# Gorilla-Lab-SCUT/frustum-convnet

Measured on AMD Instinct MI355X. Metric: frustums/sec (train fwd+bwd) KITTI-car B=32 N=1024, higher is better.
Workload: dtype f32 (fp32 operands split into two 16-bit parts, 3 MFMAs per product, fp32 accumulate); 1 GPU; cfgs/det_sample.yaml KITTI-car, batch=32/GPU, Npoint=1024, L=(280,140,70,35), train fwd+bwd+Adam; global_batch=32, parallelism=dp1

## Files before the change

frustum_convnet_amd/_native.py:

```python
import ctypes
import os

_HERE = os.path.dirname(os.path.abspath(__file__))
LIB_PATH = os.path.join(_HERE, os.environ.get("FCN_LIB_NAME", "libfcn_hip.so"))

c_fp = ctypes.c_void_p

BN_RUNNING = 0
BN_TRAIN = 1
BN_FROZEN = 2


class PnDesc(ctypes.Structure):
    _fields_ = [("B", ctypes.c_int32), ("N", ctypes.c_int32), ("L", ctypes.c_int32), ("K", ctypes.c_int32),
                ("C1", ctypes.c_int32), ("C2", ctypes.c_int32), ("C3", ctypes.c_int32),
                ("nvec", ctypes.c_int32), ("training", ctypes.c_int32),
                ("eps", ctypes.c_float), ("momentum", ctypes.c_float), ("nlc", ctypes.c_int32),
                ("precision", ctypes.c_int32), ("grouped", ctypes.c_int32)]


CN_MAXLEV = 5
CN_MAXLAYER = 18


class CnDesc(ctypes.Structure):
    _fields_ = [("B", ctypes.c_int32), ("L", ctypes.c_int32 * CN_MAXLEV), ("nvec", ctypes.c_int32),
                ("reg_out", ctypes.c_int32), ("training", ctypes.c_int32),
                ("eps", ctypes.c_float), ("momentum", ctypes.c_float), ("prepacked", ctypes.c_int32),
                ("precision", ctypes.c_int32), ("nlev", ctypes.c_int32), ("c1", ctypes.c_int32)]


class CnParams(ctypes.Structure):
    _fields_ = [("W", c_fp * CN_MAXLAYER), ("gamma", c_fp * CN_MAXLAYER), ("beta", c_fp * CN_MAXLAYER),
                ("running_mean", c_fp * CN_MAXLAYER), ("running_var", c_fp * CN_MAXLAYER),
                ("num_batches_tracked", c_fp * CN_MAXLAYER), ("bias", c_fp)]


class CnWs(ctypes.Structure):
    _fields_ = [("y", c_fp), ("dz", c_fp), ("wp", c_fp), ("bn", c_fp), ("stat", c_fp), ("bstat", c_fp),
                ("coef", c_fp), ("partial", c_fp), ("oh64", c_fp), ("flags", c_fp)]


class PnParams(ctypes.Structure):
    _fields_ = [("W", c_fp * 3), ("gamma", c_fp * 3), ("beta", c_fp * 3),
                ("running_mean", c_fp * 3), ("running_var", c_fp * 3), ("num_batches_tracked", c_fp * 3)]


class PnWs(ctypes.Structure):
    _fields_ = [("woff", c_fp), ("ent", c_fp), ("ewin", c_fp), ("tiles", c_fp), ("y2", c_fp), ("y3", c_fp), ("amax", c_fp),
                ("stat", c_fp), ("bn", c_fp), ("gmax", c_fp), ("dy3", c_fp), ("dz2", c_fp), ("bstat", c_fp),
                ("coef", c_fp), ("partial", c_fp), ("nsplit", ctypes.c_int32), ("gmom", c_fp), ("wenc", c_fp), ("flags", c_fp), ("pkey", c_fp),
                ("partial_both", ctypes.c_int32)]


class PnInferWs(ctypes.Structure):
    _fields_ = [("w1f", c_fp), ("wenc", c_fp), ("shift", c_fp)]


class InpDesc(ctypes.Structure):
    _fields_ = [("B", ctypes.c_int32), ("N", ctypes.c_int32), ("pt_stride", ctypes.c_int32), ("L", ctypes.c_int32 * 4),
                ("stride", ctypes.c_double * 4), ("max_depth", ctypes.c_double),
                ("random_flip", ctypes.c_int32), ("random_shift", ctypes.c_int32)]


class Inp5Desc(ctypes.Structure):
    _fields_ = [("B", ctypes.c_int32), ("N", ctypes.c_int32), ("pt_stride", ctypes.c_int32), ("L", ctypes.c_int32 * 5),
                ("stride", ctypes.c_double * 5), ("max_depth", ctypes.c_double),
                ("random_flip", ctypes.c_int32), ("random_shift", ctypes.c_int32)]


class InpRefineDesc(ctypes.Structure):
    _fields_ = [("B", ctypes.c_int32), ("N", ctypes.c_int32), ("pt_stride", ctypes.c_int32), ("Lpad", ctypes.c_int32 * 4),
                ("stride", ctypes.c_double * 4), ("random_flip", ctypes.c_int32), ("random_shift", ctypes.c_int32)]


EXPORTS = ("fcn_arch", "fcn_build_hash", "fcn_stat_replicas", "fcn_query_depth_point_f32", "fcn_query_depth_point_multi_f32", "fcn_pn_wgrad_rows", "fcn_pn_compact", "fcn_pn_group_compact", "fcn_pn_group_compact2",
           "fcn_pn_pack_weights", "fcn_pn_pack_weights_all", "fcn_pn_infer_fold", "fcn_pn_infer", "fcn_pn_forward", "fcn_pn_backward", "fcn_pn_backward2", "fcn_pn_backward3", "fcn_pn_backward_dense", "fcn_pn_conv_fwd", "fcn_det_loss_tail", "fcn_det_loss_tail_rows", "fcn_det_loss_tail_rows2", "fcn_det_iou_metrics",
           "fcn_det_loss_tail_scratch_floats", "fcn_adam_step_f32", "fcn_sgd_step_f32", "fcn_adam_step_slots", "fcn_prepare_inputs", "fcn_prepare_inputs_refine", "fcn_prepare_inputs_sunrgbd", "fcn_stamp", "fcn_stream_capture_id",
           "fcn_convnet_sizes", "fcn_convnet_logits_ld", "fcn_convnet_pack", "fcn_convnet_forward", "fcn_convnet_forward2",
           "fcn_convnet_backward", "fcn_box3d_iou_pair_f32", "fcn_decode_detections", "fcn_rotate_nms_3d")

_lib = None


FLAG_NONFINITE = 1


class NativeError(RuntimeError):
    pass


def lib():
    global _lib
    if _lib is not None:
        return _lib
    if not os.path.exists(LIB_PATH):
        raise ImportError(
            "frustum_convnet_amd: %s not found -- build it with `python -m frustum_convnet_amd.build` "
            "(hipcc --offload-arch=gfx950). There is no CPU/PyTorch fallback for the hot path." % LIB_PATH)
    import torch
    L = ctypes.CDLL(LIB_PATH)
    L.fcn_arch.restype = ctypes.c_int
    if hasattr(L, "fcn_build_hash"):
        L.fcn_build_hash.restype = ctypes.c_char_p
        L.fcn_build_hash.argtypes = []
    L.fcn_arch.argtypes = []
    L.fcn_pn_wgrad_rows.restype = ctypes.c_int
    L.fcn_pn_wgrad_rows.argtypes = []
    if hasattr(L, "fcn_stat_replicas"):
        L.fcn_stat_replicas.restype = ctypes.c_int
        L.fcn_stat_replicas.argtypes = []
    L.fcn_query_depth_point_f32.restype = ctypes.c_int
    L.fcn_query_depth_point_f32.argtypes = [
        c_fp, ctypes.c_int64, ctypes.c_int64, c_fp, ctypes.c_int64, ctypes.c_int64,
        ctypes.c_int, ctypes.c_int, ctypes.c_int, ctypes.c_float, ctypes.c_int, c_fp, c_fp, c_fp]
    if hasattr(L, "fcn_query_depth_point_multi_f32"):
        L.fcn_query_depth_point_multi_f32.restype = ctypes.c_int
        L.fcn_query_depth_point_multi_f32.argtypes = [ctypes.c_int, c_fp, ctypes.c_int64, ctypes.c_int64, c_fp, c_fp, c_fp,
                                                      ctypes.c_int, ctypes.c_int, c_fp, c_fp, c_fp, c_fp, c_fp, c_fp]
    L.fcn_pn_compact.restype = ctypes.c_int
    L.fcn_pn_compact.argtypes = [ctypes.POINTER(PnDesc), c_fp, c_fp, c_fp, c_fp, ctypes.POINTER(PnWs), c_fp]
    L.fcn_pn_group_compact.restype = ctypes.c_int
    L.fcn_pn_group_compact.argtypes = [ctypes.c_int, c_fp, c_fp, c_fp, c_fp, c_fp, c_fp, c_fp, c_fp]
    L.fcn_pn_group_compact2.restype = ctypes.c_int
    L.fcn_pn_group_compact2.argtypes = [ctypes.c_int, c_fp, c_fp, c_fp, c_fp, c_fp, c_fp, c_fp, ctypes.c_int, c_fp]
    if hasattr(L, "fcn_pn_pack_weights") or "FCN_LIB_NAME" not in os.environ:
        L.fcn_pn_pack_weights.restype = ctypes.c_int
        L.fcn_pn_pack_weights.argtypes = [ctypes.POINTER(PnDesc), ctypes.POINTER(PnParams), ctypes.POINTER(PnWs), c_fp]
        L.fcn_pn_pack_weights_all.restype = ctypes.c_int
        L.fcn_pn_pack_weights_all.argtypes = [ctypes.c_int, c_fp, c_fp, c_fp, c_fp]
    L.fcn_pn_forward.restype = ctypes.c_int
    L.fcn_pn_forward.argtypes = [ctypes.POINTER(PnDesc), ctypes.POINTER(PnParams), c_fp, c_fp,
                                 ctypes.POINTER(PnWs), c_fp, c_fp]
    if hasattr(L, "fcn_pn_infer") or "FCN_LIB_NAME" not in os.environ:
        L.fcn_pn_infer_fold.restype = ctypes.c_int
        L.fcn_pn_infer_fold.argtypes = [ctypes.c_int, c_fp, c_fp, c_fp, c_fp, c_fp]
        L.fcn_pn_infer.restype = ctypes.c_int
        L.fcn_pn_infer.argtypes = [ctypes.POINTER(PnDesc), c_fp, c_fp, ctypes.POINTER(PnWs), ctypes.POINTER(PnInferWs), c_fp, c_fp]
    L.fcn_pn_backward.restype = ctypes.c_int
    L.fcn_pn_backward.argtypes = [ctypes.POINTER(PnDesc), ctypes.POINTER(PnParams), c_fp,
                                  ctypes.POINTER(PnWs), c_fp * 3, c_fp * 3, c_fp * 3, c_fp]
    L.fcn_pn_backward2.restype = ctypes.c_int
    L.fcn_pn_backward2.argtypes = [ctypes.POINTER(PnDesc), ctypes.POINTER(PnParams), c_fp,
                                   ctypes.POINTER(PnWs), c_fp * 3, c_fp * 3, c_fp * 3, c_fp, c_fp, ctypes.POINTER(c_fp)]
    if hasattr(L, "fcn_pn_backward3"):
        L.fcn_pn_backward3.restype = ctypes.c_int
        L.fcn_pn_backward3.argtypes = [ctypes.POINTER(PnDesc), ctypes.POINTER(PnParams), c_fp,
                                       ctypes.POINTER(PnWs), c_fp * 3, c_fp * 3, c_fp * 3, c_fp, c_fp, c_fp, ctypes.POINTER(c_fp)]
    if hasattr(L, "fcn_pn_backward_dense"):
        L.fcn_pn_backward_dense.restype = ctypes.c_int
        L.fcn_pn_backward_dense.argtypes = [ctypes.POINTER(PnDesc), ctypes.POINTER(PnParams), c_fp,
                                            ctypes.POINTER(PnWs), c_fp * 3, c_fp * 3, c_fp * 3, c_fp]
    L.fcn_pn_conv_fwd.restype = ctypes.c_int
    L.fcn_pn_conv_fwd.argtypes = [ctypes.POINTER(PnDesc), ctypes.POINTER(PnParams), ctypes.POINTER(PnWs),
                                  ctypes.c_int, ctypes.c_int, c_fp]
    L.fcn_det_loss_tail.restype = ctypes.c_int
    L.fcn_det_loss_tail.argtypes = [c_fp] * 9 + [ctypes.c_int] * 4 + [ctypes.c_float] * 4 + [c_fp] * 4
    L.fcn_adam_step_f32.restype = ctypes.c_int
    L.fcn_adam_step_f32.argtypes = [c_fp] * 4 + [ctypes.c_int64] + [c_fp] * 3
    L.fcn_sgd_step_f32.restype = ctypes.c_int
    L.fcn_sgd_step_f32.argtypes = [c_fp] * 3 + [ctypes.c_int64] + [c_fp] * 2
    L.fcn_prepare_inputs.restype = ctypes.c_int
    L.fcn_prepare_inputs.argtypes = [ctypes.POINTER(InpDesc)] + [c_fp] * 13 + [c_fp * 4] + [c_fp] * 7
    L.fcn_prepare_inputs_sunrgbd.restype = ctypes.c_int
    L.fcn_prepare_inputs_sunrgbd.argtypes = [ctypes.POINTER(Inp5Desc)] + [c_fp] * 15 + [c_fp * 5] + [c_fp] * 7
    L.fcn_prepare_inputs_refine.restype = ctypes.c_int
    L.fcn_prepare_inputs_refine.argtypes = [ctypes.POINTER(InpRefineDesc)] + [c_fp] * 12 + [c_fp * 4] + [c_fp] * 8
    L.fcn_stamp.restype = ctypes.c_int
    L.fcn_stamp.argtypes = [c_fp, c_fp]
    L.fcn_stream_capture_id.restype = ctypes.c_int
    L.fcn_stream_capture_id.argtypes = [c_fp, ctypes.POINTER(ctypes.c_uint64)]
    L.fcn_adam_step_slots.restype = ctypes.c_int64
    L.fcn_adam_step_slots.argtypes = [ctypes.c_int64]
    L.fcn_det_loss_tail_rows.restype = ctypes.c_int
    L.fcn_det_loss_tail_rows.argtypes = [c_fp] * 8 + [ctypes.c_int] * 4 + [ctypes.c_float] * 4 + [c_fp] * 3
    L.fcn_det_loss_tail_rows2.restype = ctypes.c_int
    L.fcn_det_loss_tail_rows2.argtypes = [c_fp] * 8 + [ctypes.c_int] * 4 + [ctypes.c_float] * 4 + [c_fp] * 5
    L.fcn_det_iou_metrics.restype = ctypes.c_int
    L.fcn_det_iou_metrics.argtypes = [c_fp, ctypes.c_int] + [c_fp] * 6 + [ctypes.c_int] * 4 + [ctypes.c_float] + [c_fp] * 3
    L.fcn_det_loss_tail_scratch_floats.restype = ctypes.c_int
    L.fcn_det_loss_tail_scratch_floats.argtypes = [ctypes.c_int, ctypes.c_int]
    L.fcn_convnet_sizes.restype = ctypes.c_int
    L.fcn_convnet_sizes.argtypes = [ctypes.POINTER(CnDesc), ctypes.POINTER(ctypes.c_int64 * 6)]
    L.fcn_convnet_logits_ld.restype = ctypes.c_int
    L.fcn_convnet_logits_ld.argtypes = [ctypes.POINTER(CnDesc)]
    L.fcn_convnet_pack.restype = ctypes.c_int
    L.fcn_convnet_pack.argtypes = [ctypes.POINTER(CnDesc), ctypes.POINTER(CnParams), ctypes.POINTER(CnWs), c_fp, c_fp]
    L.fcn_convnet_forward.restype = ctypes.c_int
    L.fcn_convnet_forward.argtypes = [ctypes.POINTER(CnDesc), ctypes.POINTER(CnParams), ctypes.POINTER(CnWs),
                                      c_fp * CN_MAXLEV, c_fp, c_fp, c_fp]
    L.fcn_convnet_forward2.restype = ctypes.c_int
    L.fcn_convnet_forward2.argtypes = [ctypes.POINTER(CnDesc), ctypes.POINTER(CnParams), ctypes.POINTER(CnWs),
                                       c_fp * CN_MAXLEV, c_fp, c_fp, c_fp, ctypes.POINTER(c_fp)]
    L.fcn_convnet_backward.restype = ctypes.c_int
    L.fcn_convnet_backward.argtypes = [ctypes.POINTER(CnDesc), ctypes.POINTER(CnParams), ctypes.POINTER(CnWs),
                                       c_fp * CN_MAXLEV, c_fp, c_fp, c_fp * CN_MAXLEV, c_fp * CN_MAXLAYER, c_fp * CN_MAXLAYER,
                                       c_fp * CN_MAXLAYER, c_fp, c_fp, c_fp, ctypes.POINTER(c_fp)]
    L.fcn_box3d_iou_pair_f32.restype = ctypes.c_int
    L.fcn_box3d_iou_pair_f32.argtypes = [c_fp, c_fp, ctypes.c_int, c_fp, c_fp]
    L.fcn_decode_detections.restype = ctypes.c_int
    L.fcn_decode_detections.argtypes = [c_fp, ctypes.c_int] + [c_fp] * 5 + [ctypes.c_int] * 5 + [c_fp] * 3
    L.fcn_rotate_nms_3d.restype = ctypes.c_int
    L.fcn_rotate_nms_3d.argtypes = [c_fp] * 3 + [ctypes.c_int] * 3 + [ctypes.c_float, ctypes.c_int] + [c_fp] * 3
    _lib = L
    return L


def check(rc, what):
    if rc != 0:
        raise NativeError("%s failed with code %d (hipError_t or FCN_E_*; see include/fcn_hip.h)" % (what, rc))


def ptr(t):
    return None if t is None else ctypes.c_void_p(t.data_ptr())


def current_stream(device=None):
    import torch
    return ctypes.c_void_p(torch.cuda.current_stream(device).cuda_stream)


_unknown_capture = [0]


def capture_id(device=None):
    import torch
    if not torch.cuda.is_available() or not torch.cuda.is_current_stream_capturing():
        return 0
    cid = ctypes.c_uint64(0)
    rc = lib().fcn_stream_capture_id(current_stream(device), ctypes.byref(cid))
    if rc != 0 or cid.value == 0:
        _unknown_capture[0] -= 1
        return _unknown_capture[0]
    return int(cid.value)
```

frustum_convnet_amd/build.py:

```python
import os
import subprocess
import sys

HERE = os.path.dirname(os.path.abspath(__file__))
CSRC = os.path.join(HERE, "csrc")
SOURCES = ["grouping.hip", "group_compact.hip", "pointnet_fwd.hip", "pointnet_bwd.hip", "loss_tail.hip", "fcn_net.hip", "optim.hip", "inputs.hip", "box_iou.hip"]
HEADERS = ["fcn_common.h", "fcn_tuning.h", "gemm_tile.h", "pn_pack.h", "pn_infer.h", "box_iou.h", os.path.join("..", "..", "include", "fcn_hip.h")]
LIB = os.path.join(HERE, "libfcn_hip.so")
FLAGS = ["--offload-arch=gfx950", "-O3", "-std=c++17", "-fPIC", "-shared", "-fno-fast-math",
         "-ffp-contract=off"]


OBJ = os.path.join(CSRC, "_obj")


def source_hash(extra_flags=()):
    import hashlib
    h = hashlib.sha256()
    for name in SOURCES + HEADERS:
        with open(os.path.join(CSRC, name), "rb") as f:
            h.update(name.encode() + b"\0" + f.read() + b"\0")
    h.update(" ".join(FLAGS + list(extra_flags)).encode())
    return h.hexdigest()[:16]


def _deps_mtime():
    return max(os.path.getmtime(os.path.join(CSRC, h)) for h in HEADERS + [os.path.abspath(__file__)])


def _stale():
    if not os.path.exists(LIB):
        return True
    t = os.path.getmtime(LIB)
    deps = [os.path.join(CSRC, s) for s in SOURCES + HEADERS] + [os.path.abspath(__file__)]
    return any(os.path.getmtime(d) > t for d in deps)


def build(force=False, verbose=True, lib=None, extra_flags=()):
    variant = lib is not None or bool(extra_flags)
    lib = lib or LIB
    if not force and not variant and not _stale():
        return lib
    from concurrent.futures import ThreadPoolExecutor
    hipcc = os.environ.get("HIPCC", "/opt/rocm/bin/hipcc")
    cflags = [f for f in FLAGS if f != "-shared"] + list(extra_flags)
    objdir = OBJ + ("_variant_%d" % os.getpid() if variant else "")
    os.makedirs(objdir, exist_ok=True)
    hdr_t = _deps_mtime()

    def compile_one(src):
        path, obj = os.path.join(CSRC, src), os.path.join(objdir, src.replace(".hip", ".o"))
        if not force and not variant and os.path.exists(obj) and os.path.getmtime(obj) > max(os.path.getmtime(path), hdr_t):
            return obj
        cmd = [hipcc] + cflags + ["-c", path, "-o", obj]
        if verbose:
            print("[fcn build]", " ".join(cmd), flush=True)
        subprocess.check_call(cmd)
        return obj

    with ThreadPoolExecutor(max_workers=min(len(SOURCES), os.cpu_count() or 4)) as ex:
        objs = list(ex.map(compile_one, SOURCES))
    hsrc, hobj = os.path.join(objdir, "build_hash.cpp"), os.path.join(objdir, "build_hash.o")
    with open(hsrc, "w") as f:
        f.write('extern "C" const char *fcn_build_hash(void) { return "%s"; }\n' % source_hash(extra_flags))
    import shutil
    cxx = os.environ.get("CXX") or shutil.which("g++") or shutil.which("c++")
    if cxx:
        subprocess.check_call([cxx, "-O1", "-fPIC", "-c", hsrc, "-o", hobj])
    else:
        subprocess.check_call([hipcc, "-x", "c++", "-O1", "-fPIC", "-c", hsrc, "-o", hobj])
    objs.append(hobj)
    cmd = [hipcc, "--offload-arch=gfx950", "-shared", "-fPIC"] + objs + ["-o", lib]
    if verbose:
        print("[fcn build]", " ".join(cmd), flush=True)
    subprocess.check_call(cmd)
    if variant:
        shutil.rmtree(objdir, ignore_errors=True)
    return lib


if __name__ == "__main__":
    build(force="--force" in sys.argv)
```

frustum_convnet_amd/csrc/box_iou.hip:

```cpp
#include "fcn_common.h"
#define FCN_HD __device__ __forceinline__
#include "box_iou.h"

__global__ void iou_pair_kernel(const float *__restrict__ c1, const float *__restrict__ c2, int n, float *__restrict__ out)
{
    const int i = blockIdx.x * blockDim.x + threadIdx.x;
    if (i >= n) return;
    const float *a = c1 + (int64_t)i * 24, *b = c2 + (int64_t)i * 24;
    const int ord[4] = {6, 7, 4, 5};
    float ax[4], az[4], bx[4], bz[4];
#pragma unroll
    for (int k = 0; k < 4; ++k) {
        ax[k] = a[ord[k] * 3]; az[k] = a[ord[k] * 3 + 2];
        bx[k] = b[ord[k] * 3]; bz[k] = b[ord[k] * 3 + 2];
    }
    float i2, i3;
    fcn_iou_from_polys(ax, az, a[1], a[13], bx, bz, b[1], b[13], &i2, &i3);
    out[2 * i] = i2;
    out[2 * i + 1] = i3;
}

extern "C" int fcn_box3d_iou_pair_f32(const float *corners1, const float *corners2, int n, float *out2, void *stream)
{
    if (n < 0 || (n > 0 && (!corners1 || !corners2 || !out2))) return FCN_E_BADARG;
    if (n == 0) return 0;
    hipLaunchKernelGGL(iou_pair_kernel, dim3((n + 127) / 128), dim3(128), 0, (hipStream_t)stream, corners1, corners2, n, out2);
    FCN_CHECK_LAUNCH();
    return 0;
}

#define IOM_T 128

struct IouMetricArgs {
    const float *logits;
    const int64_t *cls_label;
    const float *ref2;
    const float *box_center, *box_heading, *box_size;
    const float *mean_size;
    float *scratch;
    float *out4;
    int B, L2, ld, nb, ns;
    float thresh;
};

__global__ __launch_bounds__(IOM_T) void iou_metric_kernel(IouMetricArgs a)
{
    __shared__ float sh[4][IOM_T / 64];
    const int tid = threadIdx.x, lane = tid & 63, wave = tid >> 6;
    const int R = a.B * a.L2, nb = a.nb, ns = a.ns;
    const int r = blockIdx.x * IOM_T + tid;
    float s2 = 0.f, s3 = 0.f, st = 0.f, sn = 0.f;
    if (r < R && a.cls_label[r] == 1) {
        const int b = r / a.L2, l = r % a.L2;
        const float *o = a.logits + (int64_t)r * a.ld + 2;
        const float per = 6.283185307179586f / (float)nb, half = per * 0.5f;
        int ah = 0, as = 0;
        float mx = o[3];
        for (int j = 1; j < nb; ++j)
            if (o[3 + j] > mx) { mx = o[3 + j]; ah = j; }
        const float *ss = o + 3 + 2 * nb;
        mx = ss[0];
        for (int j = 1; j < ns; ++j)
            if (ss[j] > mx) { mx = ss[j]; as = j; }
        float pa = (float)ah * per + o[3 + nb + ah] * half;
        if (pa > 3.141592653589793f) pa -= 6.283185307179586f;
        const float *sr3 = o + 3 + 2 * nb + ns + 3 * as;
        const float m0 = a.mean_size[as * 3], m1 = a.mean_size[as * 3 + 1], m2 = a.mean_size[as * 3 + 2];
        const float pcx = o[0] + a.ref2[((int64_t)b * 3 + 0) * a.L2 + l], pcy = o[1] + a.ref2[((int64_t)b * 3 + 1) * a.L2 + l],
                    pcz = o[2] + a.ref2[((int64_t)b * 3 + 2) * a.L2 + l];
        const float hl = a.box_heading[b];
        float i2, i3;
        fcn_iou_from_params(pcx, pcy, pcz, sr3[0] * m0 + m0, sr3[1] * m1 + m1, sr3[2] * m2 + m2, cosf(pa), sinf(pa),
                            a.box_center[b * 3], a.box_center[b * 3 + 1], a.box_center[b * 3 + 2], a.box_size[b * 3],
                            a.box_size[b * 3 + 1], a.box_size[b * 3 + 2], cosf(hl), sinf(hl), &i2, &i3);
        s2 = i2; s3 = i3; st = (i3 >= a.thresh) ? 1.f : 0.f; sn = 1.f;
    }
    s2 = wave_sum_f32(s2); s3 = wave_sum_f32(s3); st = wave_sum_f32(st); sn = wave_sum_f32(sn);
    if (lane == 0) { sh[0][wave] = s2; sh[1][wave] = s3; sh[2][wave] = st; sh[3][wave] = sn; }
    __syncthreads();
    if (tid == 0) {
        float t[4];
        for (int q = 0; q < 4; ++q) {
            t[q] = 0.f;
            for (int w = 0; w < IOM_T / 64; ++w) t[q] += sh[q][w];
            if (t[q] != 0.f) atomicAdd(&a.scratch[q], t[q]);
        }
        __threadfence();
        const int ticket = atomicAdd((int *)&a.scratch[4], 1);
        if (ticket == (int)gridDim.x - 1) {
            __threadfence();
            float v[4];
            for (int q = 0; q < 4; ++q) v[q] = __hip_atomic_load(&a.scratch[q], __ATOMIC_RELAXED, __HIP_MEMORY_SCOPE_AGENT);
            const float inv = v[3] > 0.f ? 1.f / v[3] : 0.f;
            a.out4[0] = v[0] * inv; a.out4[1] = v[1] * inv; a.out4[2] = v[2] * inv; a.out4[3] = v[3];
            for (int q = 0; q < 4; ++q) a.scratch[q] = 0.f;
            ((int *)a.scratch)[4] = 0;
        }
    }
}

extern "C" int fcn_det_iou_metrics(const float *logits, int ld, const int64_t *cls_label, const float *center_ref2,
                                   const float *box3d_center, const float *box3d_heading, const float *box3d_size,
                                   const float *mean_size, int B, int L2, int num_heading_bin, int num_size_cluster,
                                   float iou_thresh, float *scratch8, float *out4, void *stream)
{
    if (!logits || !cls_label || !center_ref2 || !box3d_center || !box3d_heading || !box3d_size || !mean_size || !scratch8 ||
        !out4)
        return FCN_E_BADARG;
    if (B <= 0 || L2 <= 0 || num_heading_bin < 1 || num_size_cluster < 1) return FCN_E_BADARG;
    if (ld < 2 + 3 + 2 * num_heading_bin + 4 * num_size_cluster) return FCN_E_BADARG;
    IouMetricArgs a;
    a.logits = logits; a.cls_label = cls_label; a.ref2 = center_ref2; a.box_center = box3d_center;
    a.box_heading = box3d_heading; a.box_size = box3d_size; a.mean_size = mean_size; a.scratch = scratch8; a.out4 = out4;
    a.B = B; a.L2 = L2; a.ld = ld; a.nb = num_heading_bin; a.ns = num_size_cluster; a.thresh = iou_thresh;
    hipLaunchKernelGGL(iou_metric_kernel, dim3((B * L2 + IOM_T - 1) / IOM_T), dim3(IOM_T), 0, (hipStream_t)stream, a);
    FCN_CHECK_LAUNCH();
    return 0;
}

#define DEC_T 256
#define DEC_NB_MAX 16
#define DEC_NS_MAX 8

struct DecodeArgs {
    const float *logits;
    const float *ref2;
    const float *mean_size;
    const float *rot_angle;
    const float *ref_center;
    const float *rgb_prob;
    float *dets;
    int32_t *valid;
    int B, L2, ld, nb, ns, method;
};

__global__ __launch_bounds__(DEC_T) void decode_kernel(DecodeArgs a)
{
    __shared__ float best_s[DEC_T];
    __shared__ int best_i[DEC_T];
    __shared__ int nfg_s;
    const int b = blockIdx.x, tid = threadIdx.x;
    const int L2 = a.L2, nb = a.nb, ns = a.ns;
    if (tid == 0) nfg_s = 0;
    __syncthreads();
    float bs = -1.f;
    int bi = 0x7fffffff, cnt = 0;
    for (int l = tid; l < L2; l += DEC_T) {
        const float *row = a.logits + ((int64_t)b * L2 + l) * a.ld;
        const float c0 = row[0], c1 = row[1];
        const float m = fmaxf(c0, c1), e0 = expf(c0 - m), e1 = expf(c1 - m);
        const float p0 = e0 / (e0 + e1), p1 = e1 / (e0 + e1);
        cnt += (p0 < p1) ? 1 : 0;
        if (p1 > bs) { bs = p1; bi = l; }
    }
    best_s[tid] = bs;
    best_i[tid] = bi;
    if (cnt) atomicAdd(&nfg_s, cnt);
    __syncthreads();
    for (int o = DEC_T / 2; o > 0; o >>= 1) {
        if (tid < o) {
            const float s2 = best_s[tid + o];
            const int i2 = best_i[tid + o];
            if (s2 > best_s[tid] || (s2 == best_s[tid] && i2 < best_i[tid])) { best_s[tid] = s2; best_i[tid] = i2; }
        }
        __syncthreads();
    }
    const bool use_top = (a.method == 0) || (nfg_s == 0);
    const int top = best_i[0];
    const float rot = a.rot_angle[b];
    const float cr = cosf(-rot), sr = sinf(-rot);
    const float rcx = a.ref_center ? a.ref_center[b * 3] : 0.f, rcy = a.ref_center ? a.ref_center[b * 3 + 1] : 0.f,
                rcz = a.ref_center ? a.ref_center[b * 3 + 2] : 0.f;
    const float rgb = a.rgb_prob ? a.rgb_prob[b] : 1.f;
    const float per = 6.283185307179586f / (float)nb, half = per * 0.5f;
    for (int l = tid; l < L2; l += DEC_T) {
        const int64_t r = (int64_t)b * L2 + l;
        const float *row = a.logits + r * a.ld;
        const float c0 = row[0], c1 = row[1];
        const float m = fmaxf(c0, c1), e0 = expf(c0 - m), e1 = expf(c1 - m);
        const float p0 = e0 / (e0 + e1), p1 = e1 / (e0 + e1);
        const bool sel = use_top ? (l == top) : (p0 < p1);
        const float *o = row + 2;
        int ah = 0, as = 0;
        float mx = o[3];
        for (int j = 1; j < nb; ++j)
            if (o[3 + j] > mx) { mx = o[3 + j]; ah = j; }
        const float *ss = o + 3 + 2 * nb;
        mx = ss[0];
        for (int j = 1; j < ns; ++j)
            if (ss[j] > mx) { mx = ss[j]; as = j; }
        float ang = (float)ah * per + o[3 + nb + ah] * half;
        if (ang > 3.141592653589793f) ang -= 6.283185307179586f;
        const float *sr3 = o + 3 + 2 * nb + ns + 3 * as;
        const float sl = sr3[0] * a.mean_size[as * 3] + a.mean_size[as * 3];
        const float sw = sr3[1] * a.mean_size[as * 3 + 1] + a.mean_size[as * 3 + 1];
        const float sh = sr3[2] * a.mean_size[as * 3 + 2] + a.mean_size[as * 3 + 2];
        const float cx = o[0] + a.ref2[((int64_t)b * 3 + 0) * L2 + l], cy = o[1] + a.ref2[((int64_t)b * 3 + 1) * L2 + l],
                    cz = o[2] + a.ref2[((int64_t)b * 3 + 2) * L2 + l];
        const float tx = cr * cx - sr * cz + rcx;
        const float tz = sr * cx + cr * cz + rcz;
        const float ty = cy + rcy + 0.5f * sh;
        float *d = a.dets + r * 8;
        d[0] = tx; d[1] = ty; d[2] = tz; d[3] = sl; d[4] = sw; d[5] = sh; d[6] = ang + rot; d[7] = p1 + rgb;
        a.valid[r] = (sel && !(sh < 0.01f || sw < 0.01f || sl < 0.01f)) ? 1 : 0;
    }
}

extern "C" int fcn_decode_detections(const float *logits, int ld, const float *center_ref2, const float *mean_size,
                                     const float *rot_angle, const float *ref_center, const float *rgb_prob, int B, int L2,
                                     int num_heading_bin, int num_size_cluster, int method, float *dets, int32_t *valid,
                                     void *stream)
{
    if (!logits || !center_ref2 || !mean_size || !rot_angle || !dets || !valid) return FCN_E_BADARG;
    if (B <= 0 || L2 <= 0 || num_heading_bin < 1 || num_size_cluster < 1) return FCN_E_BADARG;
    if (ld < 2 + 3 + 2 * num_heading_bin + 4 * num_size_cluster) return FCN_E_BADARG;
    if (method != 0 && method != 1) return FCN_E_BADARG;
    DecodeArgs a;
    a.logits = logits; a.ref2 = center_ref2; a.mean_size = mean_size; a.rot_angle = rot_angle; a.ref_center = ref_center;
    a.rgb_prob = rgb_prob; a.dets = dets; a.valid = valid; a.B = B; a.L2 = L2; a.ld = ld; a.nb = num_heading_bin;
    a.ns = num_size_cluster; a.method = method;
    hipLaunchKernelGGL(decode_kernel, dim3(B), dim3(DEC_T), 0, (hipStream_t)stream, a);
    FCN_CHECK_LAUNCH();
    return 0;
}

#define NMS_T 256
#define NMS_MAXC 4096

struct NmsArgs {
    const float *dets;
    const int32_t *valid;
    const int32_t *unit_group;
    int U, rows_per_unit, G, top_k;
    float thresh;
    int32_t *keep;
    int32_t *keep_cnt;
};

struct NmsBox {
    float x[4], z[4], ytop, ybot, lo[3], hi[3];
};

__device__ __forceinline__ void nms_load(const float *d, NmsBox &b)
{
    const float co = cosf(d[6]), si = sinf(d[6]);
    fcn_bev_rect(d[0], d[2], d[3], d[4], co, si, b.x, b.z);
    b.ytop = d[1] + 0.5f * d[5];
    b.ybot = d[1] - 0.5f * d[5];
    b.lo[0] = fminf(fminf(b.x[0], b.x[1]), fminf(b.x[2], b.x[3]));
    b.hi[0] = fmaxf(fmaxf(b.x[0], b.x[1]), fmaxf(b.x[2], b.x[3]));
    b.lo[2] = fminf(fminf(b.z[0], b.z[1]), fminf(b.z[2], b.z[3]));
    b.hi[2] = fmaxf(fmaxf(b.z[0], b.z[1]), fmaxf(b.z[2], b.z[3]));
    b.lo[1] = b.ybot;
    b.hi[1] = b.ytop;
}

__global__ __launch_bounds__(NMS_T) void nms_kernel(NmsArgs a)
{
    __shared__ float key[NMS_MAXC];
    __shared__ int32_t row[NMS_MAXC];
    __shared__ unsigned char dead[NMS_MAXC];
    __shared__ int n_s, cur_s, kept_s;
    const int g = blockIdx.x, tid = threadIdx.x;
    if (tid == 0) { n_s = 0; kept_s = 0; }
    __syncthreads();
    for (int u = 0; u < a.U; ++u) {
        if (a.unit_group[u] != g) continue;
        for (int base = 0; base < a.rows_per_unit; base += NMS_T) {
            const int l = base + tid;
            const int r = u * a.rows_per_unit + l;
            const bool ok = l < a.rows_per_unit && (!a.valid || a.valid[r] != 0);
            const unsigned long long mask = __ballot(ok);
            const int lane = tid & 63, wave = tid >> 6;
            __shared__ int wcnt[NMS_T / 64];
            if (lane == 0) wcnt[wave] = __popcll(mask);
            __syncthreads();
            int off = n_s;
            for (int w = 0; w < wave; ++w) off += wcnt[w];
            const int pos = off + __popcll(mask & ((1ull << lane) - 1ull));
            if (ok && pos < NMS_MAXC) { key[pos] = a.dets[(int64_t)r * 8 + 7]; row[pos] = r; }
            __syncthreads();
            if (tid == 0) {
                int t = 0;
                for (int w = 0; w < NMS_T / 64; ++w) t += wcnt[w];
                n_s += t;
            }
            __syncthreads();
        }
    }
    const int n = n_s;
    if (n > NMS_MAXC) {
        if (tid == 0) a.keep_cnt[g] = -1;
        return;
    }
    int np2 = 1;
    while (np2 < n) np2 <<= 1;
    for (int i = n + tid; i < np2; i += NMS_T) { key[i] = -INFINITY; row[i] = -1; }
    for (int i = tid; i < np2; i += NMS_T) dead[i] = 0;
    __syncthreads();
    for (int k = 2; k <= np2; k <<= 1) {
        for (int j = k >> 1; j > 0; j >>= 1) {
            for (int i = tid; i < np2; i += NMS_T) {
                const int p = i ^ j;
                if (p > i) {
                    const bool desc = (i & k) == 0;
                    const float ki = key[i], kp = key[p];
                    const int ri = row[i], rp = row[p];
                    const bool i_first = (ki > kp) || (ki == kp && ri > rp);
                    if (desc ? !i_first : i_first) { key[i] = kp; key[p] = ki; row[i] = rp; row[p] = ri; }
                }
            }
            __syncthreads();
        }
    }
    int i = 0;
    while (true) {
        if (tid == 0) {
            int c = i;
            while (c < n && dead[c]) ++c;
            cur_s = c;
            if (c < n) {
                if (kept_s < a.top_k) a.keep[(int64_t)g * a.top_k + kept_s] = row[c];
                kept_s += 1;
            }
        }
        __syncthreads();
        const int c = cur_s;
        if (c >= n) break;
        NmsBox bi;
        nms_load(a.dets + (int64_t)row[c] * 8, bi);
        for (int j = c + 1 + tid; j < n; j += NMS_T) {
            if (dead[j]) continue;
            NmsBox bj;
            nms_load(a.dets + (int64_t)row[j] * 8, bj);
            bool apart = false;
#pragma unroll
            for (int q = 0; q < 3; ++q) apart = apart || (fminf(bi.hi[q], bj.hi[q]) - fmaxf(bi.lo[q], bj.lo[q]) <= 0.f);
            if (apart) continue;
            float i2, i3;
            fcn_iou_from_polys(bi.x, bi.z, bi.ytop, bi.ybot, bj.x, bj.z, bj.ytop, bj.ybot, &i2, &i3);
            if (i3 >= a.thresh) dead[j] = 1;
        }
        i = c + 1;
        __syncthreads();
    }
    if (tid == 0) a.keep_cnt[g] = kept_s < a.top_k ? kept_s : a.top_k;
}

extern "C" int fcn_rotate_nms_3d(const float *dets, const int32_t *valid, const int32_t *unit_group, int num_units,
                                 int rows_per_unit, int num_groups, float thresh, int top_k, int32_t *keep,
                                 int32_t *keep_cnt, void *stream)
{
    if (!dets || !unit_group || !keep || !keep_cnt) return FCN_E_BADARG;
    if (num_units <= 0 || rows_per_unit <= 0 || num_groups <= 0 || top_k <= 0) return FCN_E_BADARG;
    NmsArgs a;
    a.dets = dets; a.valid = valid; a.unit_group = unit_group; a.U = num_units; a.rows_per_unit = rows_per_unit;
    a.G = num_groups; a.top_k = top_k; a.thresh = thresh; a.keep = keep; a.keep_cnt = keep_cnt;
    hipLaunchKernelGGL(nms_kernel, dim3(num_groups), dim3(NMS_T), 0, (hipStream_t)stream, a);
    FCN_CHECK_LAUNCH();
    return 0;
}
```

frustum_convnet_amd/csrc/loss_tail.hip:

```cpp
#include "fcn_common.h"

#define LT_NB 12
#define LT_MIN_THREADS 64

struct LossArgs {
    const float *cls_raw;
    const float *reg_raw;
    const int64_t *cls_label;
    const float *ref2;
    const float *box_center;
    const float *box_heading;
    const float *box_size;
    const int64_t *size_class;
    const float *mean_size;
    float *out;
    float *dcls;
    float *dreg;
    int B, L2;
    float w_box, w_corner, w_headreg, w_sizereg;
    int ld;
    float *scratch;
    float *total;
};

template <int NT, int N>
__device__ __forceinline__ void block_sums(float (&v)[N], float *sh)
{
    const int lane = threadIdx.x & 63, wave = threadIdx.x >> 6;
#pragma unroll
    for (int i = 0; i < N; ++i) v[i] = wave_sum_f32(v[i]);
    __syncthreads();
    if (lane == 0) {
#pragma unroll
        for (int i = 0; i < N; ++i) sh[wave * N + i] = v[i];
    }
    __syncthreads();
#pragma unroll
    for (int i = 0; i < N; ++i) {
        float t = 0.f;
        for (int w = 0; w < NT / 64; ++w) t += sh[w * N + i];
        v[i] = t;
    }
}

__device__ __forceinline__ float pymod(float a, float b) { return a - b * floorf(a / b); }

__device__ __forceinline__ void corners8(float cx, float cy, float cz, float c, float s, float l, float w, float h,
                                         float (&px)[8], float (&py)[8], float (&pz)[8])
{
#pragma unroll
    for (int k = 0; k < 8; ++k) {
        const float sx = (k & 2) ? -0.5f : 0.5f;
        const float sy = (k & 4) ? -0.5f : 0.5f;
        const float sz = ((k & 3) == 1 || (k & 3) == 2) ? -0.5f : 0.5f;
        const float x = sx * l, y = sy * h, z = sz * w;
        px[k] = c * x + s * z + cx;
        py[k] = y + cy;
        pz[k] = -s * x + c * z + cz;
    }
}

template <int NS, int LT_THREADS>
__global__ __launch_bounds__(LT_THREADS) void loss_tail_kernel(LossArgs a)
{
    constexpr int NB = LT_NB, NC = 3 + 2 * NB + 4 * NS;
    constexpr int SW = (NC + 2) | 1;
    __shared__ float shN[LT_THREADS / 64 * 11];
    __shared__ int last_s;
    __shared__ float gS[LT_THREADS * SW];
    __shared__ float gG[LT_THREADS * SW];
    const int tid = threadIdx.x;
    const int B = a.B, L2 = a.L2, R = B * L2;
    const float TWO_PI = 6.283185307179586f, PI = 3.141592653589793f;
    const float per = (float)(6.283185307179586 / NB), half = (float)(6.283185307179586 / NB / 2.0);

    typedef float lt_v4f __attribute__((ext_vector_type(4)));
    typedef const lt_v4f __attribute__((address_space(1))) *lt_gv4fp;
    constexpr int LT_NV = 16;
    const int row0 = blockIdx.x * LT_THREADS;
    const int nrow = min(LT_THREADS, R - row0);
    const int q4 = a.ld >> 2;
    const int sh_q = a.ld == 128 ? 5 : 4;
    const int nbatch = a.ld ? (q4 + LT_NV - 1) / LT_NV : 0;
    lt_v4f lv[LT_NV];
#define LT_LOAD_BATCH(bt)                                                                                             \
    _Pragma("unroll") for (int k = 0; k < LT_NV; ++k) {                                                               \
        const int i = tid + LT_THREADS * (k + LT_NV * (bt));                                                          \
        const int rr = min(i >> sh_q, nrow - 1), c4 = i & (q4 - 1);              \
        lv[k] = *(lt_gv4fp)(a.cls_raw + (int64_t)(row0 + rr) * a.ld + 4 * c4);                                        \
    }
#define LT_STAGE_BATCH(bt)                                                                                            \
    _Pragma("unroll") for (int k = 0; k < LT_NV; ++k) {                                                               \
        const int i = tid + LT_THREADS * (k + LT_NV * (bt));                                                          \
        const int rr = i >> sh_q, c4 = i & (q4 - 1);                                                                  \
        if (rr < nrow) {                                                                                              \
            _Pragma("unroll") for (int j = 0; j < 4; ++j)                                                             \
                if (4 * c4 + j < NC + 2) gS[rr * SW + 4 * c4 + j] = lv[k][j];                                         \
        }                                                                                                             \
    }
    if (a.ld) LT_LOAD_BATCH(0);

    float cfg_ = 0.f, ckeep = 0.f;
    {
        typedef long long lt_v2l __attribute__((ext_vector_type(2)));
        typedef const lt_v2l __attribute__((address_space(1))) *lt_gv2lp;
        const int R2 = R >> 1;
        constexpr int LT_CNT = 18;
        for (int base = 0; base < R2; base += LT_CNT * LT_THREADS) {
            lt_v2l lab[LT_CNT];
#pragma unroll
            for (int k = 0; k < LT_CNT; ++k) lab[k] = *(lt_gv2lp)(a.cls_label + 2 * min(base + tid + k * LT_THREADS, R2 - 1));
#pragma unroll
            for (int k = 0; k < LT_CNT; ++k) {
                const bool in = base + tid + k * LT_THREADS < R2;
                cfg_ += in ? ((lab[k][0] == 1) ? 1.f : 0.f) + ((lab[k][1] == 1) ? 1.f : 0.f) : 0.f;
                ckeep += in ? ((lab[k][0] != -1) ? 1.f : 0.f) + ((lab[k][1] != -1) ? 1.f : 0.f) : 0.f;
            }
        }
        if ((R & 1) && tid == 0) {
            const int64_t lab = a.cls_label[R - 1];
            cfg_ += (lab == 1) ? 1.f : 0.f;
            ckeep += (lab != -1) ? 1.f : 0.f;
        }
    }
    float cnt2[2] = {cfg_, ckeep};
    block_sums<LT_THREADS, 2>(cnt2, shN);
    const float nfg = cnt2[0], nkeep = cnt2[1];
    const float inv_cls = 1.f / (nfg + 1e-14f);
    const float inv_fg = nfg > 0.f ? 1.f / nfg : 0.f;

    float acc[11];
#pragma unroll
    for (int i = 0; i < 11; ++i) acc[i] = 0.f;

    if (a.ld) {
        LT_STAGE_BATCH(0);
        if (nbatch > 1) {
            LT_LOAD_BATCH(1);
            LT_STAGE_BATCH(1);
        }
        __syncthreads();
    }

    for (int r = blockIdx.x * LT_THREADS + tid; r < R; r += gridDim.x * LT_THREADS) {
        const int b = r / L2, l = r % L2;
        const int64_t lab = a.cls_label[r];
        const float c0 = a.ld ? gS[tid * SW] : a.cls_raw[((int64_t)b * 2 + 0) * L2 + l];
        const float c1 = a.ld ? gS[tid * SW + 1] : a.cls_raw[((int64_t)b * 2 + 1) * L2 + l];
        const float m = fmaxf(c0, c1);
        const float e0 = expf(c0 - m), e1 = expf(c1 - m);
        const float p0 = e0 / (e0 + e1), p1 = e1 / (e0 + e1);
        float g0 = 0.f, g1 = 0.f;
        if (lab != -1) {
            const int t = lab >= 1 ? 1 : 0;
            const float pt = t ? p1 : p0;
            const float alpha = t ? 0.25f : 0.75f;
            const float om = 1.f - pt, lg = logf(pt + 1e-14f);
            acc[1] += -alpha * om * om * lg;
            const float dpt = -alpha * (-2.f * om * lg + om * om / (pt + 1e-14f));
            const float gt_ = dpt * pt * om * inv_cls;
            g0 = t ? -gt_ : gt_;
            g1 = t ? gt_ : -gt_;
            acc[8] += ((p1 > p0 ? 1 : 0) == t) ? 1.f : 0.f;
        }
        if (a.dcls) {
            if (a.ld) {
                gG[tid * SW] = g0;
                gG[tid * SW + 1] = g1;
            } else {
                a.dcls[((int64_t)b * 2 + 0) * L2 + l] = g0;
                a.dcls[((int64_t)b * 2 + 1) * L2 + l] = g1;
            }
        }
        float *go = gG + tid * SW + 2;
#pragma unroll
        for (int j = 0; j < NC; ++j) go[j] = 0.f;
        if (lab == 1) {
            if (!a.ld) {
#pragma unroll
                for (int j = 0; j < NC; ++j) gS[tid * SW + 2 + j] = a.reg_raw[((int64_t)b * NC + j) * L2 + l];
            }
            const float *o = gS + tid * SW + 2;
            const float rx = a.ref2[((int64_t)b * 3 + 0) * L2 + l], ry = a.ref2[((int64_t)b * 3 + 1) * L2 + l],
                        rz = a.ref2[((int64_t)b * 3 + 2) * L2 + l];
            const float clx = a.box_center[b * 3], cly = a.box_center[b * 3 + 1], clz = a.box_center[b * 3 + 2];
            const float hlab = a.box_heading[b];
            const float sl0 = a.box_size[b * 3], sl1 = a.box_size[b * 3 + 1], sl2 = a.box_size[b * 3 + 2];
            const int sc = min(max((int)a.size_class[b], 0), NS - 1);
            const float ex0 = a.mean_size[sc * 3], ex1 = a.mean_size[sc * 3 + 1], ex2 = a.mean_size[sc * 3 + 2];
            const float wB = a.w_box * inv_fg;

            {
                const float dx = clx - rx - o[0], dy = cly - ry - o[1], dz = clz - rz - o[2];
                const float dist = sqrtf(dx * dx + dy * dy + dz * dz);
                const float q = fminf(dist, 3.f);
                acc[2] += 0.5f * q * q + 3.f * (dist - q);
                if (dist > 0.f) {
                    const float k = -wB * q / dist;
                    go[0] += k * dx; go[1] += k * dy; go[2] += k * dz;
                }
            }
            const float ga = pymod(hlab, TWO_PI);
            const float shifted = pymod(ga + half, TWO_PI);
            int hc = (int)floorf(shifted / per);
            hc = hc < 0 ? 0 : (hc > NB - 1 ? NB - 1 : hc);
            const float hres = (shifted - ((float)hc * per + half)) / half;
            {
                float mx = o[3];
                int am = 0;
#pragma unroll
                for (int j = 1; j < NB; ++j)
                    if (o[3 + j] > mx) { mx = o[3 + j]; am = j; }
                float se = 0.f, ej[NB];
#pragma unroll
                for (int j = 0; j < NB; ++j) { ej[j] = expf(o[3 + j] - mx); se += ej[j]; }
                acc[3] += logf(se) + mx - o[3 + hc];
#pragma unroll
                for (int j = 0; j < NB; ++j) go[3 + j] += wB * (ej[j] / se - (j == hc ? 1.f : 0.f));
                acc[9] += (am == hc) ? 1.f : 0.f;
                const float e = o[3 + NB + hc] - hres;
                const float ab = fabsf(e), q = fminf(ab, 1.f);
                acc[4] += 0.5f * q * q + (ab - q);
                go[3 + NB + hc] += wB * a.w_headreg * (e > 0.f ? q : (e < 0.f ? -q : 0.f));
            }
            {
                const float *ss = &o[3 + 2 * NB];
                float mx = ss[0];
                int am = 0;
#pragma unroll
                for (int j = 1; j < NS; ++j)
                    if (ss[j] > mx) { mx = ss[j]; am = j; }
                float se = 0.f;
#pragma unroll
                for (int j = 0; j < NS; ++j) {
                    const float ej = expf(ss[j] - mx);
                    go[3 + 2 * NB + j] = ej;
                    se += ej;
                }
                acc[5] += logf(se) + mx - ss[sc];
#pragma unroll
                for (int j = 0; j < NS; ++j) go[3 + 2 * NB + j] = wB * (go[3 + 2 * NB + j] / se - (j == sc ? 1.f : 0.f));
                acc[10] += (am == sc) ? 1.f : 0.f;
            }
            const int so = 3 + 2 * NB + NS + sc * 3;
            {
                const float v0 = (sl0 - ex0) / ex0 - o[so], v1 = (sl1 - ex1) / ex1 - o[so + 1],
                            v2 = (sl2 - ex2) / ex2 - o[so + 2];
                const float n = sqrtf(v0 * v0 + v1 * v1 + v2 * v2);
                const float q = fminf(n, 1.f);
                acc[6] += 0.5f * q * q + (n - q);
                if (n > 0.f) {
                    const float k = -wB * a.w_sizereg * q / n;
                    go[so] += k * v0; go[so + 1] += k * v1; go[so + 2] += k * v2;
                }
            }
            {
                float ang = (float)hc * per + o[3 + NB + hc] * half;
                if (ang > PI) ang -= TWO_PI;
                const float pl = o[so] * ex0 + ex0, pw = o[so + 1] * ex1 + ex1, ph = o[so + 2] * ex2 + ex2;
                const float pcx = rx + o[0], pcy = ry + o[1], pcz = rz + o[2];
                float px[8], py[8], pz[8], gx[8], gy[8], gz[8], fx[8], fy[8], fz[8];
                const float c = cosf(ang), s = sinf(ang);
                const float hf = hlab + PI;
                corners8(pcx, pcy, pcz, c, s, pl, pw, ph, px, py, pz);
                corners8(clx, cly, clz, cosf(hlab), sinf(hlab), sl0, sl1, sl2, gx, gy, gz);
                corners8(clx, cly, clz, cosf(hf), sinf(hf), sl0, sl1, sl2, fx, fy, fz);
                float d1 = 0.f, d2 = 0.f;
#pragma unroll
                for (int k = 0; k < 8; ++k) {
                    d1 += sqrtf((px[k] - gx[k]) * (px[k] - gx[k]) + (py[k] - gy[k]) * (py[k] - gy[k]) +
                                (pz[k] - gz[k]) * (pz[k] - gz[k]));
                    d2 += sqrtf((px[k] - fx[k]) * (px[k] - fx[k]) + (py[k] - fy[k]) * (py[k] - fy[k]) +
                                (pz[k] - fz[k]) * (pz[k] - fz[k]));
                }
                d1 *= 0.125f; d2 *= 0.125f;
                const bool first = d1 <= d2;
                const float cd = first ? d1 : d2;
                const float q = fminf(cd, 1.f);
                acc[7] += 0.5f * q * q + (cd - q);
                const float wk = wB * a.w_corner * q * 0.125f;
                float dcx = 0.f, dcy = 0.f, dcz = 0.f, dl = 0.f, dw = 0.f, dh = 0.f, dang = 0.f;
#pragma unroll
                for (int k = 0; k < 8; ++k) {
                    const float tx = first ? gx[k] : fx[k], ty = first ? gy[k] : fy[k], tz = first ? gz[k] : fz[k];
                    const float ex_ = px[k] - tx, ey_ = py[k] - ty, ez_ = pz[k] - tz;
                    const float nn = sqrtf(ex_ * ex_ + ey_ * ey_ + ez_ * ez_);
                    if (nn > 0.f) {
                        const float kx = wk * ex_ / nn, ky = wk * ey_ / nn, kz = wk * ez_ / nn;
                        const float sx = (k & 2) ? -0.5f : 0.5f, sy = (k & 4) ? -0.5f : 0.5f;
                        const float sz = ((k & 3) == 1 || (k & 3) == 2) ? -0.5f : 0.5f;
                        const float x = sx * pl, z = sz * pw;
                        dcx += kx; dcy += ky; dcz += kz;
                        dl += kx * c * sx - kz * s * sx;
                        dw += kx * s * sz + kz * c * sz;
                        dh += ky * sy;
                        dang += kx * (-s * x + c * z) + kz * (-c * x - s * z);
                    }
                }
                go[0] += dcx; go[1] += dcy; go[2] += dcz;
                go[so] += dl * ex0; go[so + 1] += dw * ex1; go[so + 2] += dh * ex2;
                go[3 + NB + hc] += dang * half;
            }
        }
        if (a.ld) {
        } else if (a.dreg) {
#pragma unroll
            for (int j = 0; j < NC; ++j) a.dreg[((int64_t)b * NC + j) * L2 + l] = go[j];
        }
    }
    if (a.ld && a.dcls) {
        __syncthreads();
        for (int i = tid; i < nrow * q4; i += LT_THREADS) {
            const int rr = i >> sh_q, c4 = i & (q4 - 1);
            lt_v4f v;
#pragma unroll
            for (int j = 0; j < 4; ++j) v[j] = 4 * c4 + j < NC + 2 ? gG[rr * SW + 4 * c4 + j] : 0.f;
            *(lt_v4f *)(a.dcls + (int64_t)(row0 + rr) * a.ld + 4 * c4) = v;
        }
    }
    float tot[11];
#pragma unroll
    for (int i = 0; i < 11; ++i) tot[i] = acc[i];
    block_sums<LT_THREADS, 11>(tot, shN);
    if (tid == 0) {
        int ticket;
        if (a.scratch) {
#pragma unroll
            for (int i = 1; i < 11; ++i) a.scratch[32 + 16 * blockIdx.x + i] = tot[i];
            __threadfence();
            ticket = atomicAdd((int *)a.scratch, 1);
        } else {
#pragma unroll
            for (int i = 1; i < 11; ++i) atomicAdd(&a.out[i], tot[i]);
            __threadfence();
            ticket = atomicAdd((int *)&a.out[15], 1);
        }
        last_s = (ticket == (int)gridDim.x - 1) ? 1 : 0;
    }
    __syncthreads();
    if (last_s && a.scratch) {
        __threadfence();
        float pt_[11];
#pragma unroll
        for (int i = 1; i < 11; ++i) pt_[i] = 0.f;
        for (int g = tid; g < (int)gridDim.x; g += LT_THREADS)
#pragma unroll
            for (int i = 1; i < 11; ++i)
                pt_[i] += __hip_atomic_load(&a.scratch[32 + 16 * g + i], __ATOMIC_RELAXED, __HIP_MEMORY_SCOPE_AGENT);
#pragma unroll
        for (int i = 1; i < 11; ++i) gG[tid * 11 + i] = pt_[i];
    }
    __syncthreads();
    if (last_s && tid == 0) {
        float t[11];
        if (a.scratch) {
#pragma unroll
            for (int i = 1; i < 11; ++i) t[i] = 0.f;
            const int nth = min((int)gridDim.x, LT_THREADS);
            for (int g = 0; g < nth; ++g)
#pragma unroll
                for (int i = 1; i < 11; ++i) t[i] += gG[g * 11 + i];
            ((int *)a.scratch)[0] = 0;
        } else {
            __threadfence();
#pragma unroll
            for (int i = 1; i < 11; ++i) t[i] = __hip_atomic_load(&a.out[i], __ATOMIC_RELAXED, __HIP_MEMORY_SCOPE_AGENT);
        }
        const float cls = t[1] * inv_cls;
        const float center = t[2] * inv_fg, hcls = t[3] * inv_fg, hres = t[4] * inv_fg;
        const float scls = t[5] * inv_fg, sres = t[6] * inv_fg, corner = t[7] * inv_fg;
        const float total = cls + a.w_box * (center + hcls + scls + a.w_headreg * hres + a.w_sizereg * sres + a.w_corner * corner);
        a.out[0] = total;
        a.out[1] = cls; a.out[2] = center; a.out[3] = hcls; a.out[4] = hres;
        a.out[5] = scls; a.out[6] = sres; a.out[7] = corner;
        a.out[8] = nkeep > 0.f ? t[8] / nkeep : 0.f; a.out[9] = t[9] * inv_fg; a.out[10] = t[10] * inv_fg;
        a.out[11] = nfg;
        a.out[12] = a.out[13] = a.out[14] = a.out[15] = 0.f;
        if (a.total) a.total[0] = total;
    }
}

static int launch_loss(const LossArgs &a, int ns, hipStream_t st)
{
    if (!a.scratch) {
        hipError_t e = hipMemsetAsync(a.out, 0, 16 * sizeof(float), st);
        if (e != hipSuccess) return (int)e;
    }
    const int R = a.B * a.L2;
    if (ns == 3) hipLaunchKernelGGL((loss_tail_kernel<3, 128>), dim3((R + 127) / 128), dim3(128), 0, st, a);
    else hipLaunchKernelGGL((loss_tail_kernel<10, 64>), dim3((R + 63) / 64), dim3(64), 0, st, a);
    FCN_CHECK_LAUNCH();
    return 0;
}

extern "C" int fcn_det_loss_tail(const float *cls_raw, const float *reg_raw, const int64_t *cls_label,
                                 const float *center_ref2, const float *box3d_center, const float *box3d_heading,
                                 const float *box3d_size, const int64_t *size_class, const float *mean_size,
                                 int B, int L2, int num_heading_bin, int num_size_cluster,
                                 float w_box, float w_corner, float w_headreg, float w_sizereg,
                                 float *out16, float *dcls, float *dreg, void *stream)
{
    if (!cls_raw || !reg_raw || !cls_label || !center_ref2 || !box3d_center || !box3d_heading || !box3d_size ||
        !size_class || !mean_size || !out16)
        return FCN_E_BADARG;
    if (num_heading_bin != LT_NB || (num_size_cluster != 3 && num_size_cluster != 10)) return FCN_E_LIMIT;
    if (B <= 0 || L2 <= 0) return FCN_E_BADARG;
    if ((uintptr_t)cls_label & 15) return FCN_E_BADARG;
    LossArgs a;
    a.cls_raw = cls_raw; a.reg_raw = reg_raw; a.cls_label = cls_label; a.ref2 = center_ref2;
    a.box_center = box3d_center; a.box_heading = box3d_heading; a.box_size = box3d_size; a.size_class = size_class;
    a.mean_size = mean_size; a.out = out16; a.dcls = dcls; a.dreg = dreg; a.B = B; a.L2 = L2;
    a.w_box = w_box; a.w_corner = w_corner; a.w_headreg = w_headreg; a.w_sizereg = w_sizereg; a.ld = 0;
    a.scratch = nullptr; a.total = nullptr;
    return launch_loss(a, num_size_cluster, (hipStream_t)stream);
}

extern "C" int fcn_det_loss_tail_rows2(const float *logits, const int64_t *cls_label, const float *center_ref2,
                                       const float *box3d_center, const float *box3d_heading, const float *box3d_size,
                                       const int64_t *size_class, const float *mean_size, int B, int L2,
                                       int num_heading_bin, int num_size_cluster,
                                       float w_box, float w_corner, float w_headreg, float w_sizereg,
                                       float *out16, float *dlogits, float *scratch, float *total, void *stream);

extern "C" int fcn_det_loss_tail_rows(const float *logits, const int64_t *cls_label, const float *center_ref2,
                                      const float *box3d_center, const float *box3d_heading, const float *box3d_size,
                                      const int64_t *size_class, const float *mean_size, int B, int L2,
                                      int num_heading_bin, int num_size_cluster,
                                      float w_box, float w_corner, float w_headreg, float w_sizereg,
                                      float *out16, float *dlogits, void *stream)
{
    return fcn_det_loss_tail_rows2(logits, cls_label, center_ref2, box3d_center, box3d_heading, box3d_size, size_class,
                                   mean_size, B, L2, num_heading_bin, num_size_cluster, w_box, w_corner, w_headreg,
                                   w_sizereg, out16, dlogits, nullptr, nullptr, stream);
}

extern "C" int fcn_det_loss_tail_scratch_floats(int B, int L2)
{
    return (B <= 0 || L2 <= 0) ? 0 : 32 + 16 * ((B * L2 + LT_MIN_THREADS - 1) / LT_MIN_THREADS);
}

extern "C" int fcn_det_loss_tail_rows2(const float *logits, const int64_t *cls_label, const float *center_ref2,
                                       const float *box3d_center, const float *box3d_heading, const float *box3d_size,
                                       const int64_t *size_class, const float *mean_size, int B, int L2,
                                       int num_heading_bin, int num_size_cluster,
                                       float w_box, float w_corner, float w_headreg, float w_sizereg,
                                       float *out16, float *dlogits, float *scratch, float *total, void *stream)
{
    if (!logits || !cls_label || !center_ref2 || !box3d_center || !box3d_heading || !box3d_size || !size_class ||
        !mean_size || !out16)
        return FCN_E_BADARG;
    if (num_heading_bin != LT_NB || (num_size_cluster != 3 && num_size_cluster != 10)) return FCN_E_LIMIT;
    if (B <= 0 || L2 <= 0) return FCN_E_BADARG;
    if (((uintptr_t)cls_label & 15) || ((uintptr_t)logits & 15) || ((uintptr_t)dlogits & 15)) return FCN_E_BADARG;
    LossArgs a;
    a.cls_raw = logits; a.reg_raw = nullptr; a.cls_label = cls_label; a.ref2 = center_ref2;
    a.box_center = box3d_center; a.box_heading = box3d_heading; a.box_size = box3d_size; a.size_class = size_class;
    a.mean_size = mean_size; a.out = out16; a.dcls = dlogits; a.dreg = nullptr; a.B = B; a.L2 = L2;
    a.w_box = w_box; a.w_corner = w_corner; a.w_headreg = w_headreg; a.w_sizereg = w_sizereg;
    a.ld = (2 + 3 + 2 * num_heading_bin + 4 * num_size_cluster <= 64) ? 64 : 128;
    a.scratch = scratch; a.total = total;
    return launch_loss(a, num_size_cluster, (hipStream_t)stream);
}
```

frustum_convnet_amd/det_base.py:

```python
import math

import numpy as np
import os

import torch
import torch.nn as nn
import torch.nn.functional as F

from .config import cfg
from .dataset_info import DATASET_INFO
from .common import Conv1d, Conv2d, DeConv1d, init_params, softmax_focal_loss_ignore, get_accuracy, masked_mean, bn_momentum
from .query_depth_point import QueryDepthPoint
from .pointnet_fused import WorkspacePool, pointnet_pooled, launch_pooled, attach_pooled
from . import box_ops
from . import _native


def _bn_mode(module):
    if getattr(module, "bn_frozen", False):
        return _native.BN_FROZEN
    return _native.BN_TRAIN if module.training else _native.BN_RUNNING


class PointNetModule(nn.Module):

    def __init__(self, Infea, mlp, dist, nsample, use_xyz=True, use_feature=True):
        super(PointNetModule, self).__init__()
        self.dist = dist
        self.nsample = nsample
        self.use_xyz = use_xyz
        self.use_feature = Infea > 0
        if self.use_feature or not use_xyz:
            raise NotImplementedError(
                "only the xyz-only path (Infea == 0) is implemented: every shipped cfg has "
                "WITH_EXTRA_FEAT False and train_net_det.py:296 makes Infea <= 0 otherwise")
        self.query_depth_point = QueryDepthPoint(dist, nsample)
        self.conv1 = Conv2d(Infea + 3, mlp[0], 1)
        self.conv2 = Conv2d(mlp[0], mlp[1], 1)
        self.conv3 = Conv2d(mlp[1], mlp[2], 1)
        init_params([self.conv1[0], self.conv2[0], self.conv3[0]], 'kaiming_normal')
        init_params([self.conv1[1], self.conv2[1], self.conv3[1]], 1)
        self._pool = WorkspacePool()
        self.bn_frozen = False
        self.fused_eval = os.environ.get("FCN_FUSED_EVAL", "0") != "0"

    def fuse_eval(self, flag=True):
        self.fused_eval = bool(flag)
        return self

    def freeze_bn(self, flag=True):
        self.bn_frozen = bool(flag)
        return self

    def _param_pack(self):
        convs = (self.conv1, self.conv2, self.conv3)
        params = []
        for c in convs:
            params += [c[0].weight, c[1].weight, c[1].bias]
        bufs = ([c[1].running_mean for c in convs], [c[1].running_var for c in convs],
                [c[1].num_batches_tracked for c in convs])
        return params, bufs

    def forward_pooled(self, pc, new_pc, one_hot_vec=None, nlc=False):
        params, bufs = self._param_pack()
        bn = self.conv1[1]
        feat, _, _ = pointnet_pooled(self._pool, self.dist, self.nsample, _bn_mode(self), bn.eps,
                                     bn_momentum(bn),
                                     pc.contiguous(), new_pc.contiguous(), one_hot_vec, bufs, params, nlc=nlc,
                                     fuse_eval=self.fused_eval)
        return feat

    def launch_pooled(self, pc, new_pc, one_hot_vec=None, nlc=False):
        params, bufs = self._param_pack()
        bn = self.conv1[1]
        return launch_pooled(self._pool, self.dist, self.nsample, _bn_mode(self), bn.eps,
                             bn_momentum(bn),
                             pc.contiguous(), new_pc.contiguous(), one_hot_vec, bufs, params, nlc=nlc,
                             fuse_eval=self.fused_eval)

    def prepare_pooled(self, pc, new_pc, one_hot_vec=None, nlc=False):
        from .pointnet_fused import prepare_pooled
        params, bufs = self._param_pack()
        bn = self.conv1[1]
        return prepare_pooled(self._pool, self.dist, self.nsample, _bn_mode(self), bn.eps, bn_momentum(bn),
                              pc.contiguous(), new_pc.contiguous(), one_hot_vec, bufs, params, nlc=nlc,
                              fuse_eval=self.fused_eval)

    def attach_pooled(self, handle):
        feat, _, _ = attach_pooled(self._pool, handle)
        return feat

    def front_signature(self, nlc=False):
        from .pointnet_fused import _cfg_tuple
        from . import precision as _precision
        params, bufs = self._param_pack()
        bn = self.conv1[1]
        cfgt = _cfg_tuple(self.dist, self.nsample, _bn_mode(self), bn.eps, bn_momentum(bn), params, nlc, self.fused_eval)
        return (cfgt, _precision.code(), tuple(t.data_ptr() for t in params), tuple(t.data_ptr() for b in bufs for t in b))

    def forward(self, pc, feat, new_pc=None):
        from .pointnet_fused import dense_from_entries, dense_pointnet
        params, bufs = self._param_pack()
        bn = self.conv1[1]
        if pc.requires_grad and torch.is_grad_enabled():
            raise RuntimeError("PointNetModule.forward: no gradient w.r.t. the point cloud (the reference never asks for one either: "
                               "its inputs do not require grad)")
        mode = _bn_mode(self)
        if torch.is_grad_enabled() and any(p.requires_grad for p in params):
            if mode == _native.BN_RUNNING:
                raise NotImplementedError(
                    "PointNetModule.forward in eval mode with gradients enabled and trainable parameters: the backward of "
                    "running-statistics BatchNorm is not implemented; wrap the call in torch.no_grad() (inference), call "
                    ".train() (training) or .freeze_bn() (fine-tuning through the running statistics)")
            return dense_pointnet(self._pool, self.dist, self.nsample, mode, bn.eps, bn_momentum(bn),
                                  pc.contiguous(), new_pc.contiguous(), bufs, params)
        with torch.no_grad():
            return dense_from_entries(self._pool, self.dist, self.nsample, mode, bn.eps,
                                      bn_momentum(bn),
                                      pc.contiguous(), new_pc.contiguous(), bufs, params)


class PointNetFeat(nn.Module):

    SCALES = (([64, 64, 128], 32), ([64, 64, 128], 64), ([128, 128, 256], 64), ([256, 256, 512], 128))

    def __init__(self, input_channel=3, num_vec=0):
        super(PointNetFeat, self).__init__()
        self.num_vec = num_vec
        u = cfg.DATA.HEIGHT_HALF
        assert len(u) == len(self.SCALES)
        self.num_scales = len(self.SCALES)
        for i, (mlp, nsample) in enumerate(self.SCALES):
            setattr(self, "pointnet%d" % (i + 1),
                    PointNetModule(input_channel - 3, list(mlp), u[i], nsample, use_xyz=True, use_feature=True))
        self.concurrent_scales = True
        self.fused_front = os.environ.get("FCN_FUSED_FRONT", "1") != "0"
        self._stream_cache = {}
        self._prefetched = None
        self.set_wgrad_streams((self.num_scales - 1,))
        self.bwd_share = dict(self.BWD_SHARE.get(self.num_scales, ()))
        self.share_active = False
        self._step_id = 0

    def set_wgrad_streams(self, scales, three=False):
        for k, net in enumerate(self.nets):
            net._pool.side_wgrad = k in tuple(scales)
            net._pool.side_three = bool(three) and k in tuple(scales)

    BWD_SHARE = {4: ((1, 2),), 5: ((0, 2), (1, 3))}

    def share_backward_stream(self, scale, host):
        ns = self.num_scales
        if host is None:
            self.bwd_share.pop(scale, None)
            return
        if not (0 <= scale < host < ns - 1):
            raise ValueError("share_backward_stream: need 0 <= scale < host < %d (got scale %d, host %d)" % (ns - 1, scale, host))
        self.bwd_share[scale] = host

    @property
    def nets(self):
        return tuple(getattr(self, "pointnet%d" % (i + 1)) for i in range(self.num_scales))

    def freeze_bn(self, flag=True):
        for net in self.nets:
            net.freeze_bn(flag)
        return self

    def fuse_eval(self, flag=True):
        for net in self.nets:
            net.fuse_eval(flag)
        return self

    @property
    def bn_frozen(self):
        return self.bn_mode() == _native.BN_FROZEN

    def bn_mode(self):
        flags = set(bool(getattr(net, "bn_frozen", False)) for net in self.nets)
        if len(flags) > 1:
            raise ValueError("PointNetFeat: the scales disagree on freeze_bn (%s); freeze all of them or none"
                             % [bool(net.bn_frozen) for net in self.nets])
        return _bn_mode(self.nets[0])

    def _front_key(self, point_cloud, sample_pc, one_hot_vec, nlc, training):
        ts = [point_cloud] + list(sample_pc) + ([] if one_hot_vec is None else [one_hot_vec])
        return (tuple((t.data_ptr(), tuple(t.shape), tuple(t.stride()), t._version) for t in ts), bool(nlc), int(training),
                torch.is_grad_enabled(), tuple(net.front_signature(nlc) for net in self.nets))

    def prefetch(self, point_cloud, sample_pc, one_hot_vec=None, nlc=False, before=None):
        if not (self.fused_front and self.concurrent_scales and point_cloud.is_cuda):
            return False
        self.drop_prefetch()
        from .pointnet_fused import group_compact
        dev = point_cloud.device
        nets = self.nets
        cur = torch.cuda.current_stream(dev)
        key = "pf" + str(dev)
        if key not in self._stream_cache:
            self._stream_cache[key] = (torch.cuda.Stream(device=dev), torch.cuda.Event(enable_timing=False),
                                       torch.cuda.Event(enable_timing=False))
        side, ev_in, ev_out = self._stream_cache[key]
        prepared = [nets[s].prepare_pooled(point_cloud, sample_pc[s], one_hot_vec, nlc) for s in range(self.num_scales)]
        ev_in.record(cur)
        side.wait_event(ev_in)
        with torch.cuda.stream(side):
            if before is not None:
                before()
            group_compact(prepared, point_cloud, phase=1)
            ev_out.record(side)
        for t in [point_cloud] + list(sample_pc):
            t.record_stream(side)
        self._prefetched = {"key": self._front_key(point_cloud, sample_pc, one_hot_vec, nlc, self.bn_mode()), "handles": prepared,
                            "event": ev_out, "dev": dev, "cap": _native.capture_id(dev)}
        return True

    def _prefetch_is_foreign(self):
        pf = self._prefetched
        return pf is not None and pf["cap"] != _native.capture_id(pf["dev"])

    def adopt_prefetch(self):
        pf = self._prefetched
        if pf is not None:
            pf["cap"] = _native.capture_id(pf["dev"])
            pf["event"] = None

    def join_prefetch(self):
        pf = self._prefetched
        if pf is not None and pf["event"] is not None:
            if not self._prefetch_is_foreign():
                torch.cuda.current_stream(pf["dev"]).wait_event(pf["event"])
            pf["event"] = None

    def drop_prefetch(self):
        if self._prefetched is None:
            return
        self.join_prefetch()
        for net, h in zip(self.nets, self._prefetched["handles"]):
            net._pool.release(h["ws"])
        self._prefetched = None

    def forward(self, point_cloud, sample_pc, feat=None, one_hot_vec=None, nlc=False, join=True):
        if one_hot_vec is not None:
            assert self.num_vec == one_hot_vec.shape[1]
        nets = self.nets
        ns = self.num_scales
        self.done_events = None
        mode = self.bn_mode()
        if not (self.concurrent_scales and point_cloud.is_cuda) or os.environ.get("FCN_SERIAL", "0") == "1":
            self.drop_prefetch()
            for net in nets:
                net._pool.bwd_stream = net._pool.bwd_host_pool = None
            return tuple(net.forward_pooled(point_cloud, ref, one_hot_vec, nlc) for net, ref in zip(nets, sample_pc))
        dev = point_cloud.device
        cur = torch.cuda.current_stream(dev)
        streams = self._streams(dev)
        fork = self._fork_event(dev)
        prepared = None
        if self._prefetched is not None and (self._prefetch_is_foreign() or
                                             self._prefetched["key"] != self._front_key(point_cloud, sample_pc, one_hot_vec, nlc,
                                                                                        mode)):
            self.drop_prefetch()
        if self.fused_front:
            from .pointnet_fused import group_compact, launch_prepared
            if self._prefetched is not None:
                self.join_prefetch()
                prepared = self._prefetched["handles"]
                self._prefetched = None
                group_compact(prepared, point_cloud, phase=2)
            else:
                prepared = [nets[s].prepare_pooled(point_cloud, sample_pc[s], one_hot_vec, nlc) for s in range(ns)]
                group_compact(prepared, point_cloud)
        fork.record(cur)
        sts = [streams[i] for i in range(ns - 1)] + [cur]
        self._step_id += 1
        for k in range(ns):
            host = self.bwd_share.get(k) if (self.share_active and mode != _native.BN_RUNNING) else None
            pool = nets[k]._pool
            pool.fwd_step = self._step_id
            pool.bwd_stream = None if host is None else streams[host]
            pool.bwd_host_pool = None if host is None else nets[host]._pool
        handles = [None] * ns
        for s in (ns - 1,) + tuple(range(ns - 2, 1, -1)) + (0, 1):
            if sts[s] is not cur:
                sts[s].wait_event(fork)
            with torch.cuda.stream(sts[s]):
                if prepared is not None:
                    handles[s] = launch_prepared(prepared[s])
                else:
                    handles[s] = nets[s].launch_pooled(point_cloud, sample_pc[s], one_hot_vec, nlc)
        outs = [None] * ns
        done = self._done_events(dev)
        for s in range(ns):
            with torch.cuda.stream(sts[s]):
                outs[s] = nets[s].attach_pooled(handles[s])
                done[s].record(sts[s])
        for s in range(ns):
            cur.wait_event(done[s])
            outs[s].record_stream(cur)
        return tuple(outs)

    def _done_events(self, device):
        key = "done" + str(device)
        if key not in self._stream_cache:
            self._stream_cache[key] = [torch.cuda.Event(enable_timing=False) for _ in range(self.num_scales)]
        return self._stream_cache[key]

    def _fork_event(self, device):
        key = "ev" + str(device)
        if key not in self._stream_cache:
            self._stream_cache[key] = torch.cuda.Event(enable_timing=False)
        return self._stream_cache[key]

    def _streams(self, device):
        key = str(device)
        if key not in self._stream_cache:
            self._stream_cache[key] = [torch.cuda.Stream(device=device) for _ in range(self.num_scales)]
        return self._stream_cache[key]


class ConvFeatNet(nn.Module):

    LEVELS = 4
    WIDTHS = (128, 128, 256, 512)
    DECONV_FIRST = 2

    def __init__(self, i_c=128, num_vec=3):
        super(ConvFeatNet, self).__init__()
        w = self.WIDTHS
        assert len(w) == self.LEVELS
        self.block1_conv1 = Conv1d(i_c + num_vec, w[0], 3, 1, 1)
        for j in range(2, self.LEVELS + 1):
            setattr(self, "block%d_conv1" % j, Conv1d(w[j - 2], w[j - 1], 3, 2, 1))
            setattr(self, "block%d_conv2" % j, Conv1d(w[j - 1], w[j - 1], 3, 1, 1))
            setattr(self, "block%d_merge" % j, Conv1d(w[j - 1] + w[j - 1] + num_vec, w[j - 1], 1, 1))
        levels = range(2, self.LEVELS + 1)
        for j in (levels if self.DECONV_FIRST == 2 else reversed(levels)):
            k = 1 << (j - 2)
            setattr(self, "block%d_deconv" % j, DeConv1d(w[j - 1], 256, k, k, 0))
        for m in self.modules():
            if isinstance(m, (nn.Conv1d, nn.ConvTranspose1d)):
                nn.init.kaiming_normal_(m.weight.data, mode='fan_in')
                if m.bias is not None:
                    m.bias.data.zero_()
            if isinstance(m, nn.BatchNorm1d):
                m.weight.data.fill_(1)
                m.bias.data.zero_()
        self.bn_frozen = False

    def freeze_bn(self, flag=True):
        self.bn_frozen = bool(flag)
        return self.train(self.training)

    def train(self, mode=True):
        super(ConvFeatNet, self).train(mode)
        if getattr(self, "bn_frozen", False):
            for m in self.modules():
                if isinstance(m, nn.BatchNorm1d):
                    m.train(False)
        return self

    def forward(self, *xs):
        assert len(xs) == self.LEVELS
        x = self.block1_conv1(xs[0])
        ups = []
        for j in range(2, self.LEVELS + 1):
            x = getattr(self, "block%d_conv1" % j)(x)
            x = getattr(self, "block%d_conv2" % j)(x)
            x = getattr(self, "block%d_merge" % j)(torch.cat([x, xs[j - 1]], 1))
            ups.append(getattr(self, "block%d_deconv" % j)(x))
        n = ups[0].shape[-1]
        return torch.cat([ups[0]] + [u[:, :, :n] for u in ups[1:]], 1)


class _PendingPointNetBackward:

    def __init__(self, model, feats, leaves):
        self.model, self.feats, self.leaves = model, feats, leaves

    def backward(self, scales=None):
        if any(l.grad is None for l in self.leaves):
            raise RuntimeError("phase 2 of the split backward before phase 1: differentiate the loss first")
        if not hasattr(self, "_todo"):
            self._todo = set(range(len(self.feats)))
        ks = sorted(self._todo if scales is None else set(scales))
        if not set(ks) <= self._todo:
            raise RuntimeError("scales %s were differentiated already (left: %s)" % (sorted(set(ks) - self._todo), sorted(self._todo)))
        if ks:
            torch.autograd.backward([self.feats[k] for k in ks], [self.leaves[k].grad for k in ks])
        self._todo -= set(ks)
        if self._todo:
            return
        self.model._join_side()
        if self.model._pending_split is self:
            self.model._pending_split = None
        self.feats = self.leaves = None


class PointNetDet(nn.Module):

    FEAT_NET = PointNetFeat
    CONV_NET = ConvFeatNet

    def __init__(self, input_channel=3, num_vec=0, num_classes=2):
        super(PointNetDet, self).__init__()
        dataset_name = cfg.DATA.DATASET_NAME
        assert dataset_name in DATASET_INFO
        self.category_info = DATASET_INFO[dataset_name]
        self.num_size_cluster = len(self.category_info.CLASSES)
        self.mean_size_array = self.category_info.MEAN_SIZE_ARRAY
        self.feat_net = self.FEAT_NET(input_channel, num_vec)
        self.conv_net = self.CONV_NET(128, num_vec)
        self.num_scales = self.feat_net.num_scales
        assert self.conv_net.LEVELS == self.num_scales
        self.num_classes = num_classes
        self.num_bins = cfg.DATA.NUM_HEADING_BIN
        output_size = 3 + self.num_bins * 2 + self.num_size_cluster * 4
        head_in = 256 * (self.num_scales - 1)
        self.reg_out = nn.Conv1d(head_in, output_size, 1)
        self.cls_out = nn.Conv1d(head_in, 2, 1)
        self.relu = nn.ReLU(True)
        nn.init.kaiming_uniform_(self.cls_out.weight, mode='fan_in')
        nn.init.kaiming_uniform_(self.reg_out.weight, mode='fan_in')
        self.cls_out.bias.data.zero_()
        self.reg_out.bias.data.zero_()
        self.register_buffer("_mean_size", torch.tensor(self.mean_size_array, dtype=torch.float32),
                             persistent=False)
        self.strict = False
        self.iou_fn = None
        self.fused_loss = True
        self.fused_fcn = True
        self.split_backward = False
        self._split = None
        self._pending_split = None
        self._zero_cache = {}
        self._loss_scratch = None
        from .fcn_fused import CnPool
        self._cn_pool = CnPool()
        from .loss_fused import IouMetrics
        self._iou_metrics = IouMetrics()
        self.defer_metrics_join = False
        self.last_logits = None
        self.last_logits64 = None
        self.last_num_fg = None

    def freeze_bn(self, flag=True):
        self.feat_net.freeze_bn(flag)
        self.conv_net.freeze_bn(flag)
        return self

    def fuse_eval(self, flag=True):
        self.feat_net.fuse_eval(flag)
        return self

    def _differentiates(self):
        return torch.is_grad_enabled() and (self.training or self.feat_net.bn_frozen or getattr(self.conv_net, "bn_frozen", False))

    def detect(self, data_dicts, unit_group=None, num_groups=None, method=None, thresh=None, top_k=300):
        from . import detect as fdet
        if self.training:
            raise RuntimeError("detect() runs in eval mode")
        method = cfg.TEST.METHOD if method is None else method
        thresh = cfg.TEST.THRESH if thresh is None else thresh
        dd = {k: v for k, v in data_dicts.items() if k not in ('box3d_center', 'rot_angle', 'ref_center', 'rgb_prob')}
        with torch.no_grad():
            self.forward(dd)
        if self.last_logits64 is None:
            raise RuntimeError("detect() needs the fused ConvFeatNet (fused_fcn = True)")
        refs2 = data_dicts['center_ref2']
        B, _, L2 = refs2.shape
        dev = refs2.device
        rot = data_dicts.get('rot_angle')
        rot = torch.zeros(B, device=dev) if rot is None else rot.to(dev)
        dets, valid = fdet.decode_detections(self.last_logits64, refs2, self._mean_size, rot, data_dicts.get('ref_center'),
                                             data_dicts.get('rgb_prob'), self.num_bins, self.num_size_cluster, method)
        if unit_group is None:
            unit_group = torch.arange(B, dtype=torch.int32, device=dev)
            num_groups = B
        elif num_groups is None:
            num_groups = int(unit_group.max().item()) + 1
        keep, cnt = fdet.rotate_nms_3d(dets, valid, unit_group, L2, num_groups, thresh if method == 'nms' else 2.0, top_k)
        return dets, valid, keep, cnt

    def numeric_flags(self, device=None):
        pools = [n._pool for n in self.feat_net.nets] + [self._cn_pool]
        ts = [t for pl in pools for k, t in pl._flags.items() if device is None or k == str(device)]
        if not ts:
            return torch.zeros(1, dtype=torch.int32, device=device if device is not None else self.reg_out.weight.device)
        out = ts[0].clone()
        for t in ts[1:]:
            out |= t.to(out.device)
        return out

    def check_numerics(self):
        f = int(self.numeric_flags().item())
        for pl in [n._pool for n in self.feat_net.nets] + [self._cn_pool]:
            for t in pl._flags.values():
                t.zero_()
        if f & 1:
            raise FloatingPointError("frustum_convnet_amd: a forward GEMM produced a non-finite value (fp16 operand overflow in "
                                     "split precision, |x| >= 65504, or a genuine overflow); rerun with precision 'f32' or 'bf16'")
        return f

    def prefetch(self, data_dicts, before=None):
        pc = data_dicts.get('point_cloud')
        if pc is None or not pc.is_cuda or not self.fused_fcn or data_dicts.get('one_hot') is None:
            return False
        refs = [data_dicts.get('center_ref%d' % i) for i in range(1, self.num_scales + 1)]
        xyz = pc[:, :3, :].contiguous()
        if before is not None and xyz.data_ptr() != pc.data_ptr():
            raise RuntimeError("prefetch(before=...): the batch is produced on the prefetch branch, so its point cloud must be the "
                               "(B, 3, N) tensor the front reads (a copy of the coordinate rows would be taken before it exists)")
        self._pf_xyz = ((pc.data_ptr(), tuple(pc.shape), pc._version), xyz)
        return self.feat_net.prefetch(xyz, refs, data_dicts.get('one_hot'), nlc=True, before=before)

    def _join_side(self):
        self._iou_metrics.join()
        self.feat_net.join_prefetch()

    def backward(self, loss):
        from .loss_fused import unit_grad
        if self._split is not None:
            return self.backward_split(loss)
        loss.backward(gradient=unit_grad(loss.device))
        self._join_side()

    def take_split(self):
        if self._split is None:
            raise RuntimeError("take_split needs a training forward with model.split_backward = True")
        pending = _PendingPointNetBackward(self, *self._split)
        self._split = None
        self._pending_split = pending
        return pending

    def backward_pending(self):
        return self._split is not None or self._pending_split is not None

    def backward_split(self, loss, between=None):
        from .loss_fused import unit_grad
        pending = self.take_split()
        loss.backward(gradient=unit_grad(loss.device))
        if between is not None:
            between()
        pending.backward()
        self._join_side()

    def _slice_output(self, output):
        nb, ns = self.num_bins, self.num_size_cluster
        center = output[:, 0:3]
        heading_scores = output[:, 3:3 + nb]
        heading_res_norm = output[:, 3 + nb:3 + 2 * nb]
        size_scores = output[:, 3 + 2 * nb:3 + 2 * nb + ns]
        size_res_norm = output[:, 3 + 2 * nb + ns:].reshape(output.shape[0], ns, 3)
        return center, heading_scores, heading_res_norm, size_scores, size_res_norm

    def _zero_scalar(self, like):
        key = (str(like.device), like.dtype)
        z = self._zero_cache.get(key)
        if z is None:
            z = torch.zeros((), dtype=like.dtype, device=like.device)
            self._zero_cache[key] = z
        return z

    def forward(self, data_dicts):
        point_cloud = data_dicts.get('point_cloud')
        one_hot_vec = data_dicts.get('one_hot')
        cls_label = data_dicts.get('cls_label')
        size_class_label = data_dicts.get('size_class')
        center_label = data_dicts.get('box3d_center')
        heading_label = data_dicts.get('box3d_heading')
        size_label = data_dicts.get('box3d_size')
        refs = [data_dicts.get('center_ref%d' % i) for i in range(1, self.num_scales + 1)]

        batch_size = point_cloud.shape[0]
        pf = getattr(self, "_pf_xyz", None)
        self._pf_xyz = None
        if pf is not None and pf[0] == (point_cloud.data_ptr(), tuple(point_cloud.shape), point_cloud._version):
            xyz = pf[1]
        else:
            xyz = point_cloud[:, :3, :].contiguous()
        mean_size_array = self._mean_size.to(device=point_cloud.device, dtype=point_cloud.dtype)

        logits64 = None
        self._iou_metrics.join()
        if self.backward_pending():
            self._split = self._pending_split = None
            raise RuntimeError("PointNetDet: the previous forward ran with split_backward = True and its backward was never "
                               "finished (use model.backward(loss) / backward_split(loss) / take_split().backward()): the "
                               "PointNet gradients would silently be the previous step's")
        if self.fused_fcn and not point_cloud.is_cuda:
            raise RuntimeError("frustum_convnet_amd: the hot path runs on an MI355X only (got a %s tensor); there is no "
                               "CPU fallback" % point_cloud.device)
        if self.fused_fcn and one_hot_vec is None:
            raise NotImplementedError("the fused ConvFeatNet reads the one-hot class vector (data_dicts['one_hot']); set "
                                      "model.fused_fcn = False explicitly to run the nn.Conv1d modules instead")
        if self.fused_fcn:
            from .fcn_fused import convnet_fused, convnet_prepack
            dev = point_cloud.device
            pre = convnet_prepack(self._cn_pool, self.conv_net, self.cls_out, self.reg_out, batch_size,
                                  [r.shape[2] for r in refs], one_hot_vec, dev)
            self.feat_net.share_active = True
            feats = self.feat_net(xyz, refs, None, one_hot_vec, nlc=True, join=False)
            if self.split_backward and self._differentiates():
                leaves = tuple(f.detach().requires_grad_(True) for f in feats)
                self._split = (feats, leaves)
                feats = leaves
            nxt = getattr(self, "next_batch", None)
            if nxt is not None and self._differentiates():
                self.next_batch = None
                build, self.next_batch_build = getattr(self, "next_batch_build", None), None
                self.prefetch(nxt, before=build)
            logits64 = convnet_fused(self._cn_pool, self.conv_net, self.cls_out, self.reg_out, feats, one_hot_vec, pre,
                                     self.feat_net.done_events)
            lv = logits64.view(batch_size, refs[1].shape[2], logits64.shape[1])
            nreg = self.reg_out.weight.shape[0]
            cls_raw = lv[:, :, 0:2].permute(0, 2, 1)
            reg_raw = lv[:, :, 2:2 + nreg].permute(0, 2, 1)
        else:
            self.feat_net.share_active = False
            x = self.conv_net(*self.feat_net(xyz, refs, None, one_hot_vec))
            cls_raw = self.cls_out(x)
            reg_raw = self.reg_out(x)
        self.last_logits = (cls_raw, reg_raw)
        self.last_logits64 = logits64

        num_out = reg_raw.shape[2]
        fused_tail = (center_label is not None and self.fused_loss and cls_raw.is_cuda and self.iou_fn is None
                      and not self.strict and self.num_bins == 12 and self.num_size_cluster in (3, 10))
        if not fused_tail:
            cls_scores = cls_raw.permute(0, 2, 1).reshape(-1, 2)
            outputs = reg_raw.permute(0, 2, 1).reshape(-1, reg_raw.shape[1])
            center_ref2 = refs[1].permute(0, 2, 1).reshape(-1, 3)
            cls_probs = F.softmax(cls_scores, -1)

        if center_label is None:
            assert not self.training, 'Please provide labels for training.'
            center_boxnet, heading_scores, heading_res_norm, size_scores, size_res_norm = self._slice_output(outputs)
            heading_probs = F.softmax(heading_scores, -1)
            size_probs = F.softmax(size_scores, -1)
            heading_pred_label = torch.argmax(heading_probs, -1)
            size_pred_label = torch.argmax(size_probs, -1)
            center_preds = center_boxnet + center_ref2
            heading_preds = box_ops.angle_decode(heading_res_norm, heading_pred_label, num_bins=self.num_bins)
            size_preds = box_ops.size_decode(size_res_norm, mean_size_array, size_pred_label)
            return (cls_probs.view(batch_size, -1, 2), center_preds.view(batch_size, -1, 3),
                    heading_preds.view(batch_size, -1), size_preds.view(batch_size, -1, 3),
                    heading_probs.view(batch_size, -1, self.num_bins),
                    size_probs.view(batch_size, -1, self.num_size_cluster))

        if fused_tail:
            from .loss_fused import det_loss_tail, det_loss_tail_rows, loss_scratch
            Lw = cfg.LOSS
            wts = (Lw.BOX_LOSS_WEIGHT, Lw.CORNER_LOSS_WEIGHT, Lw.HEAD_REG_WEIGHT, Lw.SIZE_REG_WEIGHT)
            if logits64 is not None:
                key = (batch_size, num_out, str(logits64.device))
                if self._loss_scratch is None or self._loss_scratch[0] != key:
                    self._loss_scratch = (key, loss_scratch(batch_size, num_out, logits64.device))
                ious = self._iou_metrics(logits64, batch_size, num_out, cls_label, refs[1], center_label, heading_label,
                                         size_label, mean_size_array, self.num_bins, self.num_size_cluster, cfg.IOU_THRESH)
                losses, (a_cls, a_head, a_size), nfg = det_loss_tail_rows(
                    logits64, batch_size, num_out, cls_label, refs[1], center_label, heading_label, size_label,
                    size_class_label, mean_size_array, self.num_bins, self.num_size_cluster, wts,
                    self._loss_scratch[1])
                if not (self.defer_metrics_join and self._differentiates()):
                    self._iou_metrics.join()
                iou2, iou3, iout = ious[0], ious[1], ious[2]
            else:
                losses, (a_cls, a_head, a_size), nfg = det_loss_tail(
                    cls_raw, reg_raw, cls_label, refs[1], center_label, heading_label, size_label, size_class_label,
                    mean_size_array, self.num_bins, self.num_size_cluster, wts)
                iou2 = iou3 = iout = self._zero_scalar(a_cls)
            self.last_num_fg = nfg
            metrics = {'cls_acc': a_cls, 'head_acc': a_head, 'size_acc': a_size, 'IoU_2D': iou2, 'IoU_3D': iou3,
                       'IoU_' + str(cfg.IOU_THRESH): iout}
            return losses, metrics

        lab = cls_label.view(-1)
        fg = (lab == 1).to(outputs.dtype)
        nfg = fg.sum()
        if self.strict:
            assert int(nfg.item()) != 0
        center_boxnet, heading_scores, heading_res_norm, size_scores, size_res_norm = self._slice_output(outputs)
        heading_probs = F.softmax(heading_scores, -1)
        size_probs = F.softmax(size_scores, -1)
        cls_loss = softmax_focal_loss_ignore(cls_probs, lab, ignore_idx=-1)

        center_lab = center_label.unsqueeze(1).expand(-1, num_out, -1).reshape(-1, 3)
        heading_lab = heading_label.expand(-1, num_out).reshape(-1)
        size_lab = size_label.unsqueeze(1).expand(-1, num_out, -1).reshape(-1, 3)
        size_cls_lab = size_class_label.expand(-1, num_out).reshape(-1)

        center_gt_offsets = box_ops.center_encode(center_lab, center_ref2)
        heading_cls_lab, heading_res_lab = box_ops.angle_encode(heading_lab, num_bins=self.num_bins)
        size_res_lab = box_ops.size_encode(size_lab, mean_size_array, size_cls_lab)

        mm = lambda v: masked_mean(v, fg, nfg)
        center_dist = torch.norm(center_gt_offsets - center_boxnet, 2, dim=-1)
        center_loss = mm(box_ops.huber_elem(center_dist, 3.0))
        heading_class_loss = mm(F.cross_entropy(heading_scores, heading_cls_lab, reduction='none'))
        hres_sel = torch.gather(heading_res_norm, 1, heading_cls_lab.view(-1, 1)).squeeze(1)
        heading_res_norm_loss = mm(box_ops.huber_elem(hres_sel - heading_res_lab, 1.0))
        size_class_loss = mm(F.cross_entropy(size_scores, size_cls_lab, reduction='none'))
        sres_sel = torch.gather(size_res_norm, 1, size_cls_lab.view(-1, 1, 1).expand(-1, 1, 3)).squeeze(1)
        size_res_norm_loss = mm(box_ops.huber_elem(torch.norm(size_res_lab - sres_sel, 2, dim=-1), 1.0))

        center_preds = box_ops.center_decode(center_ref2, center_boxnet)
        heading = box_ops.angle_decode(heading_res_norm, heading_cls_lab, num_bins=self.num_bins)
        size = box_ops.size_decode(size_res_norm, mean_size_array, size_cls_lab)
        corners_gt = box_ops.get_box3d_corners_helper(center_lab, heading_lab, size_lab)
        corners_gt_flip = box_ops.get_box3d_corners_helper(center_lab, heading_lab + np.pi, size_lab)
        corners_pred = box_ops.get_box3d_corners_helper(center_preds, heading, size)
        corners_dist = torch.min(torch.norm(corners_pred - corners_gt, 2, dim=-1).mean(-1),
                                 torch.norm(corners_pred - corners_gt_flip, 2, dim=-1).mean(-1))
        corners_loss = mm(box_ops.huber_elem(corners_dist, 1.0))

        L = cfg.LOSS
        loss = cls_loss + L.BOX_LOSS_WEIGHT * (
            center_loss + heading_class_loss + size_class_loss + L.HEAD_REG_WEIGHT * heading_res_norm_loss +
            L.SIZE_REG_WEIGHT * size_res_norm_loss + L.CORNER_LOSS_WEIGHT * corners_loss)

        with torch.no_grad():
            cls_prec = get_accuracy(cls_probs, lab, ignore=-1)
            heading_prec = get_accuracy(heading_probs, heading_cls_lab, mask=fg)
            size_prec = get_accuracy(size_probs, size_cls_lab, mask=fg)
            zero = torch.zeros((), dtype=cls_prec.dtype, device=cls_prec.device)
            iou2d_mean = iou3d_mean = iou3d_gt_mean = zero
            if self.iou_fn is not None:
                keep = fg.bool()
                hp = box_ops.angle_decode(heading_res_norm, torch.argmax(heading_probs, -1), num_bins=self.num_bins)
                sp = box_ops.size_decode(size_res_norm, mean_size_array, torch.argmax(size_probs, -1))
                cp = box_ops.get_box3d_corners_helper(center_preds, hp, sp)
                ov = self.iou_fn(cp[keep].detach().cpu().numpy(), corners_gt[keep].detach().cpu().numpy())
                iou2d_mean = torch.tensor(ov[:, 0].mean()).type_as(cls_prec)
                iou3d_mean = torch.tensor(ov[:, 1].mean()).type_as(cls_prec)
                iou3d_gt_mean = torch.tensor((ov[:, 1] >= cfg.IOU_THRESH).mean()).type_as(cls_prec)

        losses = {'total_loss': loss, 'cls_loss': cls_loss, 'center_loss': center_loss,
                  'head_cls_loss': heading_class_loss, 'head_res_loss': heading_res_norm_loss,
                  'size_cls_loss': size_class_loss, 'size_res_loss': size_res_norm_loss,
                  'corners_loss': corners_loss}
        metrics = {'cls_acc': cls_prec, 'head_acc': heading_prec, 'size_acc': size_prec,
                   'IoU_2D': iou2d_mean, 'IoU_3D': iou3d_mean, 'IoU_' + str(cfg.IOU_THRESH): iou3d_gt_mean}
        return losses, metrics
```

frustum_convnet_amd/loss_fused.py:

```python
import torch

from . import _native


_UNIT = {}


def unit_grad(device):
    key = str(device)
    if key not in _UNIT:
        _UNIT[key] = torch.ones((), dtype=torch.float32, device=device)
    return _UNIT[key]


def _is_unit(g):
    u = _UNIT.get(str(g.device))
    return u is not None and g.data_ptr() == u.data_ptr()


def _check_labels(cls_label, size_class, ns):
    if cls_label.dtype != torch.int64 or size_class.dtype != torch.int64:
        raise TypeError("cls_label / size_class must be int64 (got %s / %s)" % (cls_label.dtype, size_class.dtype))

LOSS_NAMES = ("total_loss", "cls_loss", "center_loss", "head_cls_loss", "head_res_loss", "size_cls_loss",
              "size_res_loss", "corners_loss")


class _LossTail(torch.autograd.Function):
    @staticmethod
    def forward(ctx, cls_raw, reg_raw, cls_label, ref2, center, heading, size, size_class, mean_size, nb, ns, w):
        L = _native.lib()
        _check_labels(cls_label, size_class, ns)
        B, _, L2 = cls_raw.shape
        cls_c, reg_c = cls_raw.detach().contiguous(), reg_raw.detach().contiguous()
        need = cls_raw.requires_grad or reg_raw.requires_grad
        out = torch.empty(16, dtype=torch.float32, device=cls_raw.device)
        dcls = torch.empty_like(cls_c) if need else None
        dreg = torch.empty_like(reg_c) if need else None
        args = [cls_label.contiguous(), ref2.contiguous().float(), center.contiguous().float(),
                heading.contiguous().float(), size.contiguous().float(), size_class.contiguous(),
                mean_size.contiguous().float()]
        with torch.cuda.device(cls_raw.device):
            rc = L.fcn_det_loss_tail(cls_c.data_ptr(), reg_c.data_ptr(), *[t.data_ptr() for t in args],
                                     B, L2, int(nb), int(ns), float(w[0]), float(w[1]), float(w[2]), float(w[3]),
                                     out.data_ptr(), None if dcls is None else dcls.data_ptr(),
                                     None if dreg is None else dreg.data_ptr(), _native.current_stream(cls_raw.device))
        _native.check(rc, "fcn_det_loss_tail")
        ctx.save_for_backward(*(t for t in (dcls, dreg) if t is not None))
        ctx.need = need
        total = out[0].clone()
        rest = out.detach()
        ctx.mark_non_differentiable(rest)
        return total, rest

    @staticmethod
    def backward(ctx, gtotal, _grest):
        if not ctx.need:
            return (None,) * 12
        dcls, dreg = ctx.saved_tensors
        return (dcls * gtotal, dreg * gtotal) + (None,) * 10


def det_loss_tail(cls_raw, reg_raw, cls_label, center_ref2, box3d_center, box3d_heading, box3d_size, size_class,
                  mean_size, num_bins, num_sizes, weights):
    if not cls_raw.is_cuda:
        raise RuntimeError("frustum_convnet_amd: fused loss tail runs on the GPU only")
    total, rest = _LossTail.apply(cls_raw, reg_raw, cls_label, center_ref2, box3d_center, box3d_heading, box3d_size,
                                  size_class, mean_size, num_bins, num_sizes, weights)
    losses = {"total_loss": total}
    for i, k in enumerate(LOSS_NAMES[1:], start=1):
        losses[k] = rest[i]
    return losses, (rest[8], rest[9], rest[10]), rest[11]


class _LossTailRows(torch.autograd.Function):

    @staticmethod
    def forward(ctx, logits, cls_label, ref2, center, heading, size, size_class, mean_size, B, L2, nb, ns, w, scratch):
        L = _native.lib()
        _check_labels(cls_label, size_class, ns)
        lg = logits.detach().contiguous()
        need = logits.requires_grad
        out = torch.empty(16, dtype=torch.float32, device=lg.device)
        total = torch.empty((), dtype=torch.float32, device=lg.device)
        dlog = torch.empty_like(lg) if need else None
        args = [cls_label.contiguous(), ref2.contiguous().float(), center.contiguous().float(),
                heading.contiguous().float(), size.contiguous().float(), size_class.contiguous(),
                mean_size.contiguous().float()]
        with torch.cuda.device(lg.device):
            rc = L.fcn_det_loss_tail_rows2(lg.data_ptr(), *[t.data_ptr() for t in args], int(B), int(L2), int(nb),
                                           int(ns), float(w[0]), float(w[1]), float(w[2]), float(w[3]),
                                           out.data_ptr(), None if dlog is None else dlog.data_ptr(),
                                           None if scratch is None else scratch.data_ptr(), total.data_ptr(),
                                           _native.current_stream(lg.device))
        _native.check(rc, "fcn_det_loss_tail_rows2")
        ctx.need = need
        if need:
            ctx.save_for_backward(dlog)
        ctx.mark_non_differentiable(out)
        ctx.set_materialize_grads(False)
        return total, out

    @staticmethod
    def backward(ctx, gtotal, _grest):
        if not ctx.need or gtotal is None:
            return (None,) * 14
        (dlog,) = ctx.saved_tensors
        return (dlog if _is_unit(gtotal) else dlog * gtotal,) + (None,) * 13


def loss_scratch(B, L2, device):
    n = int(_native.lib().fcn_det_loss_tail_scratch_floats(int(B), int(L2)))
    return torch.zeros(max(n, 32), dtype=torch.float32, device=device)


def det_loss_tail_rows(logits, B, L2, cls_label, center_ref2, box3d_center, box3d_heading, box3d_size, size_class,
                       mean_size, num_bins, num_sizes, weights, scratch=None):
    total, rest = _LossTailRows.apply(logits, cls_label, center_ref2, box3d_center, box3d_heading, box3d_size,
                                      size_class, mean_size, B, L2, num_bins, num_sizes, weights, scratch)
    losses = {"total_loss": total}
    for i, k in enumerate(LOSS_NAMES[1:], start=1):
        losses[k] = rest[i]
    return losses, (rest[8], rest[9], rest[10]), rest[11]


class IouMetrics:

    def __init__(self):
        self.per_dev = {}
        self._join = None

    def __call__(self, logits, B, L2, cls_label, center_ref2, box3d_center, box3d_heading, box3d_size, mean_size, num_bins,
                 num_sizes, iou_thresh):
        dev = logits.device
        key = str(dev)
        if key not in self.per_dev:
            with torch.cuda.device(dev):
                self.per_dev[key] = (torch.cuda.Stream(device=dev), torch.cuda.Event(enable_timing=False),
                                     torch.cuda.Event(enable_timing=False),
                                     torch.zeros(8, dtype=torch.float32, device=dev))
        side, ev_in, ev_out, scratch = self.per_dev[key]
        if cls_label.dtype != torch.int64:
            raise TypeError("cls_label must be int64 (got %s)" % cls_label.dtype)
        lg = logits.detach()
        out = torch.empty(4, dtype=torch.float32, device=dev)
        args = [cls_label.contiguous(), center_ref2.contiguous().float(), box3d_center.contiguous().float(),
                box3d_heading.contiguous().float(), box3d_size.contiguous().float(), mean_size.contiguous().float()]
        cur = torch.cuda.current_stream(dev)
        ev_in.record(cur)
        side.wait_event(ev_in)
        with torch.cuda.stream(side):
            with torch.cuda.device(dev):
                rc = _native.lib().fcn_det_iou_metrics(lg.data_ptr(), int(lg.shape[1]), *[t.data_ptr() for t in args], int(B),
                                                       int(L2), int(num_bins), int(num_sizes), float(iou_thresh),
                                                       scratch.data_ptr(), out.data_ptr(), _native.current_stream(dev))
            _native.check(rc, "fcn_det_iou_metrics")
            ev_out.record(side)
        for t in [lg, out] + args:
            t.record_stream(side)
        self._join = (cur, ev_out)
        return out

    def join(self):
        if self._join is not None:
            cur, ev = self._join
            cur.wait_event(ev)
            self._join = None
```

include/fcn_hip.h:

```cpp
#ifndef FCN_HIP_H
#define FCN_HIP_H

#include <stdint.h>

#ifdef __cplusplus
extern "C" {
#endif

#define FCN_E_BADARG 10001
#define FCN_E_LIMIT  10002

#define FCN_PREC_SPLIT 0
#define FCN_PREC_F32   1
#define FCN_PREC_BF16  2
#define FCN_PREC_BF16_OPS 3

int fcn_arch(void);

int fcn_query_depth_point_f32(const float *pts_z, int64_t pt_stride, int64_t pt_bstride,
                              const float *ctr_z, int64_t ct_stride, int64_t ct_bstride,
                              int b, int n, int m, float dis_z, int nsample,
                              int64_t *idx, int32_t *cnt, void *stream);

int fcn_query_depth_point_multi_f32(int nscale, const float *pts_z, int64_t pt_stride, int64_t pt_bstride,
                                    const float *const *ctr_z, const int64_t *ct_stride, const int64_t *ct_bstride,
                                    int b, int n, const int32_t *m, const float *dis_z, const int32_t *nsample,
                                    int64_t *const *idx, int32_t *const *cnt, void *stream);

#define FCN_BN_RUNNING 0
#define FCN_BN_TRAIN   1
#define FCN_BN_FROZEN  2

typedef struct fcn_pn_desc {
    int32_t B, N, L, K;
    int32_t C1, C2, C3;
    int32_t nvec;
    int32_t training;
    float   eps, momentum;
    int32_t nlc;
    int32_t precision;
    int32_t grouped;
} fcn_pn_desc;

typedef struct fcn_pn_params {
    const float *W[3];
    const float *gamma[3], *beta[3];
    float *running_mean[3], *running_var[3];
    int64_t *num_batches_tracked[3];
} fcn_pn_params;

typedef struct fcn_pn_ws {
    int32_t *woff;
    float   *ent;
    int32_t *ewin;
    int32_t *tiles;
    float   *y2;
    float   *y3;
    int32_t *amax;
    double  *stat;
    float   *bn;
    float   *gmax;
    float   *dy3;
    float   *dz2;
    double  *bstat;
    float   *coef;
    float   *partial;
    int32_t  nsplit;
    double  *gmom;
    float   *wenc;
    int32_t *flags;
    uint64_t *pkey;
    int32_t  partial_both;
} fcn_pn_ws;

#define FCN_FLAG_NONFINITE 1

int fcn_pn_wgrad_rows(void);
int fcn_stat_replicas(void);

int fcn_pn_compact(const fcn_pn_desc *d, const float *pc , const float *ref ,
                   const int64_t *idx, const int32_t *cnt, const fcn_pn_ws *ws, void *stream);

int fcn_pn_group_compact(int nscale, const fcn_pn_desc *const *d, const fcn_pn_params *const *p, const float *pc,
                         const float *const *ref, const float *dis_z, const fcn_pn_ws *const *ws, int32_t *const *cnt,
                         void *stream);

int fcn_pn_group_compact2(int nscale, const fcn_pn_desc *const *d, const fcn_pn_params *const *p, const float *pc,
                          const float *const *ref, const float *dis_z, const fcn_pn_ws *const *ws, int32_t *const *cnt,
                          int phase, void *stream);

int fcn_pn_pack_weights(const fcn_pn_desc *d, const fcn_pn_params *p, const fcn_pn_ws *ws, void *stream);
int fcn_pn_pack_weights_all(int nscale, const fcn_pn_desc *const *d, const fcn_pn_params *const *p,
                            const fcn_pn_ws *const *ws, void *stream);

int fcn_pn_forward(const fcn_pn_desc *d, const fcn_pn_params *p, const int32_t *cnt,
                   const float *one_hot, const fcn_pn_ws *ws, float *feat, void *stream);

int fcn_pn_backward(const fcn_pn_desc *d, const fcn_pn_params *p, const float *dfeat,
                    const fcn_pn_ws *ws, float *dW[3], float *dgamma[3], float *dbeta[3], void *stream);

int fcn_pn_backward2(const fcn_pn_desc *d, const fcn_pn_params *p, const float *dfeat,
                     const fcn_pn_ws *ws, float *dW[3], float *dgamma[3], float *dbeta[3],
                     void *stream, void *stream2, void *const *events);

int fcn_pn_backward_dense(const fcn_pn_desc *d, const fcn_pn_params *p, const float *dz3,
                          const fcn_pn_ws *ws, float *dW[3], float *dgamma[3], float *dbeta[3], void *stream);

int fcn_pn_backward3(const fcn_pn_desc *d, const fcn_pn_params *p, const float *dfeat,
                     const fcn_pn_ws *ws, float *dW[3], float *dgamma[3], float *dbeta[3],
                     void *stream, void *stream2, void *stream3, void *const *events);

typedef struct fcn_pn_infer_ws {
    float *w1f;
    float *wenc;
    float *shift;
} fcn_pn_infer_ws;
int fcn_pn_infer_fold(int nscale, const fcn_pn_desc *const *d, const fcn_pn_params *const *p,
                      const fcn_pn_infer_ws *const *iws, float *const *feat, void *stream);
int fcn_pn_infer(const fcn_pn_desc *d, const int32_t *cnt, const float *one_hot, const fcn_pn_ws *ws,
                 const fcn_pn_infer_ws *iws, float *feat, void *stream);

int fcn_pn_conv_fwd(const fcn_pn_desc *d, const fcn_pn_params *p, const fcn_pn_ws *ws, int layer,
                    int with_stats, void *stream);

#define FCN_CN_MAXLEV 5
#define FCN_CN_MAXLAYER 18

typedef struct fcn_cn_desc {
    int32_t B;
    int32_t L[FCN_CN_MAXLEV];
    int32_t nvec;
    int32_t reg_out;
    int32_t training;
    float   eps, momentum;
    int32_t prepacked;
    int32_t precision;
    int32_t nlev;
    int32_t c1;
} fcn_cn_desc;

typedef struct fcn_cn_params {
    const float *W[FCN_CN_MAXLAYER];
    const float *gamma[FCN_CN_MAXLAYER], *beta[FCN_CN_MAXLAYER];
    float *running_mean[FCN_CN_MAXLAYER], *running_var[FCN_CN_MAXLAYER];
    int64_t *num_batches_tracked[FCN_CN_MAXLAYER];
    const float *bias;
} fcn_cn_params;

typedef struct fcn_cn_ws {
    float  *y, *dz, *wp, *bn;
    double *stat, *bstat;
    float  *coef, *partial;
    float  *oh64;
    int32_t *flags;
} fcn_cn_ws;

int fcn_convnet_sizes(const fcn_cn_desc *d, int64_t *out6);
int fcn_convnet_pack(const fcn_cn_desc *d, const fcn_cn_params *p, const fcn_cn_ws *ws, const float *one_hot, void *stream);
int fcn_convnet_logits_ld(const fcn_cn_desc *d);
int fcn_convnet_forward(const fcn_cn_desc *d, const fcn_cn_params *p, const fcn_cn_ws *ws,
                        const float *const feats[FCN_CN_MAXLEV], const float *one_hot, float *logits, void *stream);
int fcn_convnet_forward2(const fcn_cn_desc *d, const fcn_cn_params *p, const fcn_cn_ws *ws,
                         const float *const feats[FCN_CN_MAXLEV], const float *one_hot, float *logits, void *stream,
                         void *const *feat_events);
int fcn_convnet_backward(const fcn_cn_desc *d, const fcn_cn_params *p, const fcn_cn_ws *ws,
                         const float *const feats[FCN_CN_MAXLEV], const float *one_hot, const float *dlogits,
                         float *const dfeats[FCN_CN_MAXLEV], float *const dW[FCN_CN_MAXLAYER],
                         float *const dgamma[FCN_CN_MAXLAYER], float *const dbeta[FCN_CN_MAXLAYER], float *dbias,
                         void *stream, void *stream2, void *const *events);

int fcn_det_loss_tail(const float *cls_raw, const float *reg_raw, const int64_t *cls_label,
                      const float *center_ref2, const float *box3d_center, const float *box3d_heading,
                      const float *box3d_size, const int64_t *size_class, const float *mean_size,
                      int B, int L2, int num_heading_bin, int num_size_cluster,
                      float w_box, float w_corner, float w_headreg, float w_sizereg,
                      float *out16, float *dcls, float *dreg, void *stream);
int fcn_det_loss_tail_rows(const float *logits, const int64_t *cls_label, const float *center_ref2,
                           const float *box3d_center, const float *box3d_heading, const float *box3d_size,
                           const int64_t *size_class, const float *mean_size, int B, int L2,
                           int num_heading_bin, int num_size_cluster,
                           float w_box, float w_corner, float w_headreg, float w_sizereg,
                           float *out16, float *dlogits, void *stream);

int64_t fcn_adam_step_slots(int64_t n);
int fcn_adam_step_f32(float *param, const float *grad, float *exp_avg, float *exp_avg_sq, int64_t n,
                      const float *hyper6, int64_t *step_slots, void *stream);

int fcn_sgd_step_f32(float *param, const float *grad, float *momentum_buf, int64_t n, const float *hyper4, void *stream);

int fcn_det_loss_tail_scratch_floats(int B, int L2);
int fcn_det_loss_tail_rows2(const float *logits, const int64_t *cls_label, const float *center_ref2,
                            const float *box3d_center, const float *box3d_heading, const float *box3d_size,
                            const int64_t *size_class, const float *mean_size, int B, int L2,
                            int num_heading_bin, int num_size_cluster,
                            float w_box, float w_corner, float w_headreg, float w_sizereg,
                            float *out16, float *dlogits, float *scratch, float *total, void *stream);

int fcn_box3d_iou_pair_f32(const float *corners1, const float *corners2, int n, float *out2, void *stream);
int fcn_det_iou_metrics(const float *logits, int ld, const int64_t *cls_label, const float *center_ref2,
                        const float *box3d_center, const float *box3d_heading, const float *box3d_size,
                        const float *mean_size, int B, int L2, int num_heading_bin, int num_size_cluster,
                        float iou_thresh, float *scratch8, float *out4, void *stream);
int fcn_decode_detections(const float *logits, int ld, const float *center_ref2, const float *mean_size,
                          const float *rot_angle, const float *ref_center, const float *rgb_prob, int B, int L2,
                          int num_heading_bin, int num_size_cluster, int method, float *dets, int32_t *valid,
                          void *stream);
int fcn_rotate_nms_3d(const float *dets, const int32_t *valid, const int32_t *unit_group, int num_units, int rows_per_unit,
                      int num_groups, float thresh, int top_k, int32_t *keep, int32_t *keep_cnt, void *stream);

int fcn_stamp(uint64_t *slot, void *stream);

int fcn_stream_capture_id(void *stream, uint64_t *id);

const char *fcn_build_hash(void);


typedef struct fcn_inp_desc {
    int32_t B, N, pt_stride;
    int32_t L[4];
    double  stride[4], max_depth;
    int32_t random_flip, random_shift;
} fcn_inp_desc;
int fcn_prepare_inputs(const fcn_inp_desc *d, const float *raw_pts, const int64_t *pt_off, const int64_t *raw_seg,
                       const int32_t *choice, const double *frustum_angle, const double *box2d, const double *P,
                       const double *box3d_corners, const double *heading, const double *size,
                       const double *coin, const double *normal, float *point_cloud, float *const center_ref[4],
                       int64_t *cls_label, float *box3d_center, float *box3d_heading, float *box3d_size,
                       float *rot_angle, int64_t *seg_label, void *stream);

typedef struct fcn_inp5_desc {
    int32_t B, N, pt_stride;
    int32_t L[5];
    double  stride[5], max_depth;
    int32_t random_flip, random_shift;
} fcn_inp5_desc;
int fcn_prepare_inputs_sunrgbd(const fcn_inp5_desc *d, const float *raw_pts, const int64_t *pt_off, const int64_t *raw_seg,
                               const int32_t *choice, const double *frustum_angle, const double *box2d, const double *K,
                               const double *Rtilt, const double *box3d_corners, const double *heading, const double *size,
                               const double *coin, const double *normal, const double *hshift, float *point_cloud,
                               float *const center_ref[5], int64_t *cls_label, float *box3d_center, float *box3d_heading,
                               float *box3d_size, float *rot_angle, int64_t *seg_label, void *stream);

typedef struct fcn_inp_refine_desc {
    int32_t B, N, pt_stride;
    int32_t Lpad[4];
    double  stride[4];
    int32_t random_flip, random_shift;
} fcn_inp_refine_desc;
int fcn_prepare_inputs_refine(const fcn_inp_refine_desc *d, const float *raw_pts, const int64_t *pt_off,
                              const int32_t *choice, const double *pred_corners, const double *pred_angle,
                              const double *pred_size, const double *box3d_corners, const double *heading,
                              const double *size, const double *coin, const double *normal, float *point_cloud,
                              float *const center_ref[4], int64_t *cls_label, float *box3d_center, float *box3d_heading,
                              float *box3d_size, float *rot_angle, float *ref_center, int32_t *lens, void *stream);

#ifdef __cplusplus
}
#endif
#endif
```

Measured before the change: 29670 frustums/s.

## Defer loss-tail final combine into side-stream IoU metrics kernel

The loss tail kernel can now skip its final reduction of per-block partial sums (defer mode). That combine step moves into an extra block of the IoU metrics kernel, which runs on a side stream. The loss computation is now launched before the IoU metrics so the metrics kernel can finish the loss outputs. The aim is to take the last-block combine off the critical path of the main stream. In exchange, the loss scalars are only valid once the side stream has joined, which adds a cross-stream dependency on the loss outputs.

```diff
diff --git a/frustum_convnet_amd/_native.py b/frustum_convnet_amd/_native.py
--- a/frustum_convnet_amd/_native.py
+++ b/frustum_convnet_amd/_native.py
@@ -75,7 +75,7 @@
 
 
 EXPORTS = ("fcn_arch", "fcn_build_hash", "fcn_stat_replicas", "fcn_query_depth_point_f32", "fcn_query_depth_point_multi_f32", "fcn_pn_wgrad_rows", "fcn_pn_compact", "fcn_pn_group_compact", "fcn_pn_group_compact2",
-           "fcn_pn_pack_weights", "fcn_pn_pack_weights_all", "fcn_pn_infer_fold", "fcn_pn_infer", "fcn_pn_forward", "fcn_pn_backward", "fcn_pn_backward2", "fcn_pn_backward3", "fcn_pn_backward_dense", "fcn_pn_conv_fwd", "fcn_det_loss_tail", "fcn_det_loss_tail_rows", "fcn_det_loss_tail_rows2", "fcn_det_iou_metrics",
+           "fcn_pn_pack_weights", "fcn_pn_pack_weights_all", "fcn_pn_infer_fold", "fcn_pn_infer", "fcn_pn_forward", "fcn_pn_backward", "fcn_pn_backward2", "fcn_pn_backward3", "fcn_pn_backward_dense", "fcn_pn_conv_fwd", "fcn_det_loss_tail", "fcn_det_loss_tail_rows", "fcn_det_loss_tail_rows2", "fcn_det_loss_tail_rows3", "fcn_det_iou_metrics", "fcn_det_iou_metrics2",
            "fcn_det_loss_tail_scratch_floats", "fcn_adam_step_f32", "fcn_sgd_step_f32", "fcn_adam_step_slots", "fcn_prepare_inputs", "fcn_prepare_inputs_refine", "fcn_prepare_inputs_sunrgbd", "fcn_stamp", "fcn_stream_capture_id",
            "fcn_convnet_sizes", "fcn_convnet_logits_ld", "fcn_convnet_pack", "fcn_convnet_forward", "fcn_convnet_forward2",
            "fcn_convnet_backward", "fcn_box3d_iou_pair_f32", "fcn_decode_detections", "fcn_rotate_nms_3d")
@@ -176,6 +176,11 @@
     L.fcn_det_loss_tail_rows.argtypes = [c_fp] * 8 + [ctypes.c_int] * 4 + [ctypes.c_float] * 4 + [c_fp] * 3
     L.fcn_det_loss_tail_rows2.restype = ctypes.c_int
     L.fcn_det_loss_tail_rows2.argtypes = [c_fp] * 8 + [ctypes.c_int] * 4 + [ctypes.c_float] * 4 + [c_fp] * 5
+    L.fcn_det_loss_tail_rows3.restype = ctypes.c_int
+    L.fcn_det_loss_tail_rows3.argtypes = [c_fp] * 8 + [ctypes.c_int] * 4 + [ctypes.c_float] * 4 + [c_fp] * 4 + [ctypes.c_int, c_fp]
+    L.fcn_det_iou_metrics2.restype = ctypes.c_int
+    L.fcn_det_iou_metrics2.argtypes = ([c_fp, ctypes.c_int] + [c_fp] * 6 + [ctypes.c_int] * 4 + [ctypes.c_float] + [c_fp] * 5 +
+                                       [ctypes.c_float] * 4 + [c_fp])
     L.fcn_det_iou_metrics.restype = ctypes.c_int
     L.fcn_det_iou_metrics.argtypes = [c_fp, ctypes.c_int] + [c_fp] * 6 + [ctypes.c_int] * 4 + [ctypes.c_float] + [c_fp] * 3
     L.fcn_det_loss_tail_scratch_floats.restype = ctypes.c_int
diff --git a/frustum_convnet_amd/build.py b/frustum_convnet_amd/build.py
--- a/frustum_convnet_amd/build.py
+++ b/frustum_convnet_amd/build.py
@@ -5,7 +5,7 @@
 HERE = os.path.dirname(os.path.abspath(__file__))
 CSRC = os.path.join(HERE, "csrc")
 SOURCES = ["grouping.hip", "group_compact.hip", "pointnet_fwd.hip", "pointnet_bwd.hip", "loss_tail.hip", "fcn_net.hip", "optim.hip", "inputs.hip", "box_iou.hip"]
-HEADERS = ["fcn_common.h", "fcn_tuning.h", "gemm_tile.h", "pn_pack.h", "pn_infer.h", "box_iou.h", os.path.join("..", "..", "include", "fcn_hip.h")]
+HEADERS = ["fcn_common.h", "fcn_tuning.h", "gemm_tile.h", "pn_pack.h", "pn_infer.h", "box_iou.h", "loss_combine.h", os.path.join("..", "..", "include", "fcn_hip.h")]
 LIB = os.path.join(HERE, "libfcn_hip.so")
 FLAGS = ["--offload-arch=gfx950", "-O3", "-std=c++17", "-fPIC", "-shared", "-fno-fast-math",
          "-ffp-contract=off"]
diff --git a/frustum_convnet_amd/csrc/box_iou.hip b/frustum_convnet_amd/csrc/box_iou.hip
--- a/frustum_convnet_amd/csrc/box_iou.hip
+++ b/frustum_convnet_amd/csrc/box_iou.hip
@@ -1,6 +1,7 @@
 #include "fcn_common.h"
 #define FCN_HD __device__ __forceinline__
 #include "box_iou.h"
+#include "loss_combine.h"
 
 __global__ void iou_pair_kernel(const float *__restrict__ c1, const float *__restrict__ c2, int n, float *__restrict__ out)
 {
@@ -41,14 +42,25 @@
     float *out4;
     int B, L2, ld, nb, ns;
     float thresh;
+    const float *lt_scratch;
+    float *lt_out, *lt_total;
+    LossWeights lw;
 };
 
 __global__ __launch_bounds__(IOM_T) void iou_metric_kernel(IouMetricArgs a)
 {
     __shared__ float sh[4][IOM_T / 64];
+    __shared__ float lt_lds[128 * 11];
     const int tid = threadIdx.x, lane = tid & 63, wave = tid >> 6;
     const int R = a.B * a.L2, nb = a.nb, ns = a.ns;
-    const int r = blockIdx.x * IOM_T + tid;
+    const int extra = a.lt_scratch ? 1 : 0;
+    if (extra && blockIdx.x == 0) {
+        const int *hd = (const int *)a.lt_scratch;
+        lt_combine(a.lt_scratch, hd[3], min(hd[4], 128), hd[5], a.lt_scratch[1], a.lt_scratch[2], lt_lds, a.lt_out, a.lt_total,
+                   a.lw, tid, IOM_T);
+        return;
+    }
+    const int r = ((int)blockIdx.x - extra) * IOM_T + tid;
     float s2 = 0.f, s3 = 0.f, st = 0.f, sn = 0.f;
     if (r < R && a.cls_label[r] == 1) {
         const int b = r / a.L2, l = r % a.L2;
@@ -87,7 +99,7 @@
         }
         __threadfence();
         const int ticket = atomicAdd((int *)&a.scratch[4], 1);
-        if (ticket == (int)gridDim.x - 1) {
+        if (ticket == (int)gridDim.x - extra - 1) {
             __threadfence();
             float v[4];
             for (int q = 0; q < 4; ++q) v[q] = __hip_atomic_load(&a.scratch[q], __ATOMIC_RELAXED, __HIP_MEMORY_SCOPE_AGENT);
@@ -104,6 +116,19 @@
                                    const float *mean_size, int B, int L2, int num_heading_bin, int num_size_cluster,
                                    float iou_thresh, float *scratch8, float *out4, void *stream)
 {
+    return fcn_det_iou_metrics2(logits, ld, cls_label, center_ref2, box3d_center, box3d_heading, box3d_size, mean_size, B, L2,
+                                num_heading_bin, num_size_cluster, iou_thresh, scratch8, out4, nullptr, nullptr, nullptr, 0.f, 0.f,
+                                0.f, 0.f, stream);
+}
+
+extern "C" int fcn_det_iou_metrics2(const float *logits, int ld, const int64_t *cls_label, const float *center_ref2,
+                                    const float *box3d_center, const float *box3d_heading, const float *box3d_size,
+                                    const float *mean_size, int B, int L2, int num_heading_bin, int num_size_cluster,
+                                    float iou_thresh, float *scratch8, float *out4, const float *loss_scratch,
+                                    float *loss_out16, float *loss_total, float w_box, float w_corner, float w_headreg,
+                                    float w_sizereg, void *stream)
+{
+    if (loss_scratch && !loss_out16) return FCN_E_BADARG;
     if (!logits || !cls_label || !center_ref2 || !box3d_center || !box3d_heading || !box3d_size || !mean_size || !scratch8 ||
         !out4)
         return FCN_E_BADARG;
@@ -113,7 +138,10 @@
     a.logits = logits; a.cls_label = cls_label; a.ref2 = center_ref2; a.box_center = box3d_center;
     a.box_heading = box3d_heading; a.box_size = box3d_size; a.mean_size = mean_size; a.scratch = scratch8; a.out4 = out4;
     a.B = B; a.L2 = L2; a.ld = ld; a.nb = num_heading_bin; a.ns = num_size_cluster; a.thresh = iou_thresh;
-    hipLaunchKernelGGL(iou_metric_kernel, dim3((B * L2 + IOM_T - 1) / IOM_T), dim3(IOM_T), 0, (hipStream_t)stream, a);
+    a.lt_scratch = loss_scratch; a.lt_out = loss_out16; a.lt_total = loss_total;
+    a.lw.w_box = w_box; a.lw.w_corner = w_corner; a.lw.w_headreg = w_headreg; a.lw.w_sizereg = w_sizereg;
+    hipLaunchKernelGGL(iou_metric_kernel, dim3((B * L2 + IOM_T - 1) / IOM_T + (loss_scratch ? 1 : 0)), dim3(IOM_T), 0,
+                       (hipStream_t)stream, a);
     FCN_CHECK_LAUNCH();
     return 0;
 }
diff --git a/frustum_convnet_amd/csrc/loss_combine.h b/frustum_convnet_amd/csrc/loss_combine.h
--- /dev/null
+++ b/frustum_convnet_amd/csrc/loss_combine.h
@@ -0,0 +1,56 @@
+#pragma once
+
+struct LossWeights {
+    float w_box, w_corner, w_headreg, w_sizereg;
+};
+
+__device__ __forceinline__ void lt_combine(const float *scratch, int G, int tref, int pair, float nfg, float nkeep, float *lds,
+                                           float *out, float *total_out, LossWeights w, int tid, int nthr)
+{
+    const int Gv = pair ? (G + 1) >> 1 : G;
+    const int nth = Gv < tref ? Gv : tref;
+    __syncthreads();
+    for (int g = tid; g < nth; g += nthr) {
+        float pt_[11];
+#pragma unroll
+        for (int i = 1; i < 11; ++i) pt_[i] = 0.f;
+        for (int h = g; h < Gv; h += tref) {
+#pragma unroll
+            for (int i = 1; i < 11; ++i) {
+                float v;
+                if (pair) {
+                    v = __hip_atomic_load(&scratch[32 + 16 * (2 * h) + i], __ATOMIC_RELAXED, __HIP_MEMORY_SCOPE_AGENT);
+                    v += (2 * h + 1 < G)
+                             ? __hip_atomic_load(&scratch[32 + 16 * (2 * h + 1) + i], __ATOMIC_RELAXED, __HIP_MEMORY_SCOPE_AGENT)
+                             : 0.f;
+                } else {
+                    v = __hip_atomic_load(&scratch[32 + 16 * h + i], __ATOMIC_RELAXED, __HIP_MEMORY_SCOPE_AGENT);
+                }
+                pt_[i] += v;
+            }
+        }
+#pragma unroll
+        for (int i = 1; i < 11; ++i) lds[g * 11 + i] = pt_[i];
+    }
+    __syncthreads();
+    if (tid != 0) return;
+    float t[11];
+#pragma unroll
+    for (int i = 1; i < 11; ++i) t[i] = 0.f;
+    for (int g = 0; g < nth; ++g)
+#pragma unroll
+        for (int i = 1; i < 11; ++i) t[i] += lds[g * 11 + i];
+    const float inv_cls = 1.f / (nfg + 1e-14f);
+    const float inv_fg = nfg > 0.f ? 1.f / nfg : 0.f;
+    const float cls = t[1] * inv_cls;
+    const float center = t[2] * inv_fg, hcls = t[3] * inv_fg, hres = t[4] * inv_fg;
+    const float scls = t[5] * inv_fg, sres = t[6] * inv_fg, corner = t[7] * inv_fg;
+    const float total = cls + w.w_box * (center + hcls + scls + w.w_headreg * hres + w.w_sizereg * sres + w.w_corner * corner);
+    out[0] = total;
+    out[1] = cls; out[2] = center; out[3] = hcls; out[4] = hres;
+    out[5] = scls; out[6] = sres; out[7] = corner;
+    out[8] = nkeep > 0.f ? t[8] / nkeep : 0.f; out[9] = t[9] * inv_fg; out[10] = t[10] * inv_fg;
+    out[11] = nfg;
+    out[12] = out[13] = out[14] = out[15] = 0.f;
+    if (total_out) total_out[0] = total;
+}
diff --git a/frustum_convnet_amd/csrc/loss_tail.hip b/frustum_convnet_amd/csrc/loss_tail.hip
--- a/frustum_convnet_amd/csrc/loss_tail.hip
+++ b/frustum_convnet_amd/csrc/loss_tail.hip
@@ -1,4 +1,5 @@
 #include "fcn_common.h"
+#include "loss_combine.h"
 
 #define LT_NB 12
 #define LT_MIN_THREADS 64
@@ -21,6 +22,7 @@
     int ld;
     float *scratch;
     float *total;
+    int defer;
 };
 
 template <int NT, int N>
@@ -60,19 +62,155 @@
     }
 }
 
-template <int NS, int LT_THREADS>
+template <int NS>
+__device__ __forceinline__ void lt_fg_row(const LossArgs &a, const float *o, float *go, int b, int l, float inv_fg, int lane,
+                                          float (&lv)[8])
+{
+    constexpr int NB = LT_NB;
+    const int L2 = a.L2;
+    const float TWO_PI = 6.283185307179586f, PI = 3.141592653589793f;
+    const float per = (float)(6.283185307179586 / NB), half = (float)(6.283185307179586 / NB / 2.0);
+    const float rx = a.ref2[((int64_t)b * 3 + 0) * L2 + l], ry = a.ref2[((int64_t)b * 3 + 1) * L2 + l],
+                rz = a.ref2[((int64_t)b * 3 + 2) * L2 + l];
+    const float clx = a.box_center[b * 3], cly = a.box_center[b * 3 + 1], clz = a.box_center[b * 3 + 2];
+    const float hlab = a.box_heading[b];
+    const float sl0 = a.box_size[b * 3], sl1 = a.box_size[b * 3 + 1], sl2 = a.box_size[b * 3 + 2];
+    const int sc = min(max((int)a.size_class[b], 0), NS - 1);
+    const float ex0 = a.mean_size[sc * 3], ex1 = a.mean_size[sc * 3 + 1], ex2 = a.mean_size[sc * 3 + 2];
+    const float wB = a.w_box * inv_fg;
+
+    float gc0 = 0.f, gc1 = 0.f, gc2 = 0.f;
+    {
+        const float dx = clx - rx - o[0], dy = cly - ry - o[1], dz = clz - rz - o[2];
+        const float dist = sqrtf(dx * dx + dy * dy + dz * dz);
+        const float q = fminf(dist, 3.f);
+        lv[0] = 0.5f * q * q + 3.f * (dist - q);
+        if (dist > 0.f) {
+            const float k = -wB * q / dist;
+            gc0 += k * dx; gc1 += k * dy; gc2 += k * dz;
+        }
+    }
+    const float ga = pymod(hlab, TWO_PI);
+    const float shifted = pymod(ga + half, TWO_PI);
+    int hc = (int)floorf(shifted / per);
+    hc = hc < 0 ? 0 : (hc > NB - 1 ? NB - 1 : hc);
+    const float hres = (shifted - ((float)hc * per + half)) / half;
+    const float *ss = &o[3 + 2 * NB];
+    float mx = o[3], mxs = ss[0];
+    int am = 0, ams = 0;
+#pragma unroll
+    for (int j = 1; j < NB; ++j)
+        if (o[3 + j] > mx) { mx = o[3 + j]; am = j; }
+#pragma unroll
+    for (int j = 1; j < NS; ++j)
+        if (ss[j] > mxs) { mxs = ss[j]; ams = j; }
+    const bool isH = lane < NB, isS = lane >= NB && lane < NB + NS;
+    const float xin = o[isH ? 3 + lane : (isS ? 3 + 2 * NB + (lane - NB) : 3)];
+    const float ev = expf(xin - (isH ? mx : (isS ? mxs : xin)));
+    float se = 0.f, ses = 0.f;
+#pragma unroll
+    for (int j = 0; j < NB; ++j) se += __shfl(ev, j, 64);
+#pragma unroll
+    for (int j = 0; j < NS; ++j) ses += __shfl(ev, NB + j, 64);
+    lv[1] = logf(se) + mx - o[3 + hc];
+    lv[6] = (am == hc) ? 1.f : 0.f;
+    lv[3] = logf(ses) + mxs - ss[sc];
+    lv[7] = (ams == sc) ? 1.f : 0.f;
+    if (isH) go[3 + lane] = 0.f + wB * (ev / se - (lane == hc ? 1.f : 0.f));
+    if (isS) go[3 + 2 * NB + (lane - NB)] = wB * (ev / ses - ((lane - NB) == sc ? 1.f : 0.f));
+    float ghr = 0.f;
+    {
+        const float e = o[3 + NB + hc] - hres;
+        const float ab = fabsf(e), q = fminf(ab, 1.f);
+        lv[2] = 0.5f * q * q + (ab - q);
+        ghr += wB * a.w_headreg * (e > 0.f ? q : (e < 0.f ? -q : 0.f));
+    }
+    const int so = 3 + 2 * NB + NS + sc * 3;
+    float gs0 = 0.f, gs1 = 0.f, gs2 = 0.f;
+    {
+        const float v0 = (sl0 - ex0) / ex0 - o[so], v1 = (sl1 - ex1) / ex1 - o[so + 1], v2 = (sl2 - ex2) / ex2 - o[so + 2];
+        const float n = sqrtf(v0 * v0 + v1 * v1 + v2 * v2);
+        const float q = fminf(n, 1.f);
+        lv[4] = 0.5f * q * q + (n - q);
+        if (n > 0.f) {
+            const float k = -wB * a.w_sizereg * q / n;
+            gs0 += k * v0; gs1 += k * v1; gs2 += k * v2;
+        }
+    }
+    float ang = (float)hc * per + o[3 + NB + hc] * half;
+    if (ang > PI) ang -= TWO_PI;
+    const float pl = o[so] * ex0 + ex0, pw = o[so + 1] * ex1 + ex1, ph = o[so + 2] * ex2 + ex2;
+    const float pcx = rx + o[0], pcy = ry + o[1], pcz = rz + o[2];
+    const float hf = hlab + PI;
+    const int lt = lane < 3 ? lane : lane - 3;
+    const float A = lt == 0 ? ang : (lt == 1 ? hlab : hf);
+    float tr = 0.f;
+    if (lane < 3) tr = cosf(A);
+    else if (lane < 6) tr = sinf(A);
+    const float c = __shfl(tr, 0, 64), cg = __shfl(tr, 1, 64), cf = __shfl(tr, 2, 64);
+    const float s = __shfl(tr, 3, 64), sg = __shfl(tr, 4, 64), sf = __shfl(tr, 5, 64);
+    const int k = lane & 7;
+    const bool flip = (lane & 8) != 0;
+    const float sx = (k & 2) ? -0.5f : 0.5f;
+    const float sy = (k & 4) ? -0.5f : 0.5f;
+    const float sz = ((k & 3) == 1 || (k & 3) == 2) ? -0.5f : 0.5f;
+    const float x = sx * pl, y = sy * ph, z = sz * pw;
+    const float px = c * x + s * z + pcx, py = y + pcy, pz = -s * x + c * z + pcz;
+    const float tc = flip ? cf : cg, ts = flip ? sf : sg;
+    const float xt = sx * sl0, yt = sy * sl2, zt = sz * sl1;
+    const float tx = tc * xt + ts * zt + clx, ty = yt + cly, tz = -ts * xt + tc * zt + clz;
+    const float ex_ = px - tx, ey_ = py - ty, ez_ = pz - tz;
+    const float nn = sqrtf(ex_ * ex_ + ey_ * ey_ + ez_ * ez_);
+    float d1 = 0.f, d2 = 0.f;
+#pragma unroll
+    for (int j = 0; j < 8; ++j) {
+        d1 += __shfl(nn, j, 64);
+        d2 += __shfl(nn, 8 + j, 64);
+    }
+    d1 *= 0.125f; d2 *= 0.125f;
+    const bool first = d1 <= d2;
+    const float cd = first ? d1 : d2;
+    const float q = fminf(cd, 1.f);
+    lv[5] = 0.5f * q * q + (cd - q);
+    const float wk = wB * a.w_corner * q * 0.125f;
+    const float kx = wk * ex_ / nn, ky = wk * ey_ / nn, kz = wk * ez_ / nn;
+    const float t_l = kx * c * sx - kz * s * sx;
+    const float t_w = kx * s * sz + kz * c * sz;
+    const float t_h = ky * sy;
+    const float t_a = kx * (-s * x + c * z) + kz * (-c * x - s * z);
+    const int base = first ? 0 : 8;
+    float dcx = 0.f, dcy = 0.f, dcz = 0.f, dl = 0.f, dw = 0.f, dh = 0.f, dang = 0.f;
+#pragma unroll
+    for (int j = 0; j < 8; ++j) {
+        const float n_j = __shfl(nn, base + j, 64);
+        const float a0 = __shfl(kx, base + j, 64), a1 = __shfl(ky, base + j, 64), a2 = __shfl(kz, base + j, 64);
+        const float a3 = __shfl(t_l, base + j, 64), a4 = __shfl(t_w, base + j, 64), a5 = __shfl(t_h, base + j, 64);
+        const float a6 = __shfl(t_a, base + j, 64);
+        if (n_j > 0.f) {
+            dcx += a0; dcy += a1; dcz += a2;
+            dl += a3; dw += a4; dh += a5; dang += a6;
+        }
+    }
+    if (lane == 0) {
+        go[0] = gc0 + dcx; go[1] = gc1 + dcy; go[2] = gc2 + dcz;
+        go[so] = gs0 + dl * ex0; go[so + 1] = gs1 + dw * ex1; go[so + 2] = gs2 + dh * ex2;
+        go[3 + NB + hc] = ghr + dang * half;
+    }
+}
+
+template <int NS, int LT_THREADS, int TREF>
 __global__ __launch_bounds__(LT_THREADS) void loss_tail_kernel(LossArgs a)
 {
     constexpr int NB = LT_NB, NC = 3 + 2 * NB + 4 * NS;
     constexpr int SW = (NC + 2) | 1;
+    constexpr int PAIR = (LT_THREADS == 64 && TREF == 128) ? 1 : 0;
+    static_assert(TREF * 11 <= LT_THREADS * SW, "the combine's per-thread sums are parked in gG");
     __shared__ float shN[LT_THREADS / 64 * 11];
     __shared__ int last_s;
     __shared__ float gS[LT_THREADS * SW];
     __shared__ float gG[LT_THREADS * SW];
-    const int tid = threadIdx.x;
+    const int tid = threadIdx.x, lane = tid & 63;
     const int B = a.B, L2 = a.L2, R = B * L2;
-    const float TWO_PI = 6.283185307179586f, PI = 3.141592653589793f;
-    const float per = (float)(6.283185307179586 / NB), half = (float)(6.283185307179586 / NB / 2.0);
 
     typedef float lt_v4f __attribute__((ext_vector_type(4)));
     typedef const lt_v4f __attribute__((address_space(1))) *lt_gv4fp;
@@ -100,6 +238,12 @@
     }
     if (a.ld) LT_LOAD_BATCH(0);
 
+    const int r = row0 + tid;
+    const bool live = r < R;
+    const int b = live ? r / L2 : 0, l = live ? r % L2 : 0;
+    const int64_t lab = live ? a.cls_label[r] : (int64_t)-1;
+    const bool fg = live && lab == 1;
+
     float cfg_ = 0.f, ckeep = 0.f;
     {
         typedef long long lt_v2l __attribute__((ext_vector_type(2)));
@@ -107,20 +251,20 @@
         const int R2 = R >> 1;
         constexpr int LT_CNT = 18;
         for (int base = 0; base < R2; base += LT_CNT * LT_THREADS) {
-            lt_v2l lab[LT_CNT];
-#pragma unroll
-            for (int k = 0; k < LT_CNT; ++k) lab[k] = *(lt_gv2lp)(a.cls_label + 2 * min(base + tid + k * LT_THREADS, R2 - 1));
+            lt_v2l lab2[LT_CNT];
+#pragma unroll
+            for (int k = 0; k < LT_CNT; ++k) lab2[k] = *(lt_gv2lp)(a.cls_label + 2 * min(base + tid + k * LT_THREADS, R2 - 1));
 #pragma unroll
             for (int k = 0; k < LT_CNT; ++k) {
                 const bool in = base + tid + k * LT_THREADS < R2;
-                cfg_ += in ? ((lab[k][0] == 1) ? 1.f : 0.f) + ((lab[k][1] == 1) ? 1.f : 0.f) : 0.f;
-                ckeep += in ? ((lab[k][0] != -1) ? 1.f : 0.f) + ((lab[k][1] != -1) ? 1.f : 0.f) : 0.f;
+                cfg_ += in ? ((lab2[k][0] == 1) ? 1.f : 0.f) + ((lab2[k][1] == 1) ? 1.f : 0.f) : 0.f;
+                ckeep += in ? ((lab2[k][0] != -1) ? 1.f : 0.f) + ((lab2[k][1] != -1) ? 1.f : 0.f) : 0.f;
             }
         }
         if ((R & 1) && tid == 0) {
-            const int64_t lab = a.cls_label[R - 1];
-            cfg_ += (lab == 1) ? 1.f : 0.f;
-            ckeep += (lab != -1) ? 1.f : 0.f;
+            const int64_t labl = a.cls_label[R - 1];
+            cfg_ += (labl == 1) ? 1.f : 0.f;
+            ckeep += (labl != -1) ? 1.f : 0.f;
         }
     }
     float cnt2[2] = {cfg_, ckeep};
@@ -133,18 +277,23 @@
 #pragma unroll
     for (int i = 0; i < 11; ++i) acc[i] = 0.f;
 
+    if (live) {
+#pragma unroll
+        for (int j = 0; j < NC; ++j) gG[tid * SW + 2 + j] = 0.f;
+    }
     if (a.ld) {
         LT_STAGE_BATCH(0);
         if (nbatch > 1) {
             LT_LOAD_BATCH(1);
             LT_STAGE_BATCH(1);
         }
-        __syncthreads();
-    }
-
-    for (int r = blockIdx.x * LT_THREADS + tid; r < R; r += gridDim.x * LT_THREADS) {
-        const int b = r / L2, l = r % L2;
-        const int64_t lab = a.cls_label[r];
+    } else if (fg) {
+#pragma unroll
+        for (int j = 0; j < NC; ++j) gS[tid * SW + 2 + j] = a.reg_raw[((int64_t)b * NC + j) * L2 + l];
+    }
+    __syncthreads();
+
+    if (live) {
         const float c0 = a.ld ? gS[tid * SW] : a.cls_raw[((int64_t)b * 2 + 0) * L2 + l];
         const float c1 = a.ld ? gS[tid * SW + 1] : a.cls_raw[((int64_t)b * 2 + 1) * L2 + l];
         const float m = fmaxf(c0, c1);
@@ -172,156 +321,52 @@
                 a.dcls[((int64_t)b * 2 + 1) * L2 + l] = g1;
             }
         }
-        float *go = gG + tid * SW + 2;
-#pragma unroll
-        for (int j = 0; j < NC; ++j) go[j] = 0.f;
-        if (lab == 1) {
-            if (!a.ld) {
-#pragma unroll
-                for (int j = 0; j < NC; ++j) gS[tid * SW + 2 + j] = a.reg_raw[((int64_t)b * NC + j) * L2 + l];
+    }
+    {
+        unsigned long long todo = __ballot(fg);
+        while (todo != 0ull) {
+            const int src = __builtin_ctzll(todo);
+            todo &= todo - 1ull;
+            const int rr = (tid & ~63) + src, rw = row0 + rr;
+            float v[8];
+            lt_fg_row<NS>(a, gS + rr * SW + 2, gG + rr * SW + 2, rw / L2, rw % L2, inv_fg, lane, v);
+            if (lane == src) {
+                acc[2] += v[0]; acc[3] += v[1]; acc[4] += v[2]; acc[5] += v[3]; acc[6] += v[4]; acc[7] += v[5];
+                acc[9] += v[6]; acc[10] += v[7];
             }
-            const float *o = gS + tid * SW + 2;
-            const float rx = a.ref2[((int64_t)b * 3 + 0) * L2 + l], ry = a.ref2[((int64_t)b * 3 + 1) * L2 + l],
-                        rz = a.ref2[((int64_t)b * 3 + 2) * L2 + l];
-            const float clx = a.box_center[b * 3], cly = a.box_center[b * 3 + 1], clz = a.box_center[b * 3 + 2];
-            const float hlab = a.box_heading[b];
-            const float sl0 = a.box_size[b * 3], sl1 = a.box_size[b * 3 + 1], sl2 = a.box_size[b * 3 + 2];
-            const int sc = min(max((int)a.size_class[b], 0), NS - 1);
-            const float ex0 = a.mean_size[sc * 3], ex1 = a.mean_size[sc * 3 + 1], ex2 = a.mean_size[sc * 3 + 2];
-            const float wB = a.w_box * inv_fg;
-
-            {
-                const float dx = clx - rx - o[0], dy = cly - ry - o[1], dz = clz - rz - o[2];
-                const float dist = sqrtf(dx * dx + dy * dy + dz * dz);
-                const float q = fminf(dist, 3.f);
-                acc[2] += 0.5f * q * q + 3.f * (dist - q);
-                if (dist > 0.f) {
-                    const float k = -wB * q / dist;
-                    go[0] += k * dx; go[1] += k * dy; go[2] += k * dz;
-                }
+        }
+    }
+    __syncthreads();
+    if (a.ld) {
+        if (a.dcls) {
+            for (int i = tid; i < nrow * q4; i += LT_THREADS) {
+                const int rr = i >> sh_q, c4 = i & (q4 - 1);
+                lt_v4f v;
+#pragma unroll
+                for (int j = 0; j < 4; ++j) v[j] = 4 * c4 + j < NC + 2 ? gG[rr * SW + 4 * c4 + j] : 0.f;
+                *(lt_v4f *)(a.dcls + (int64_t)(row0 + rr) * a.ld + 4 * c4) = v;
             }
-            const float ga = pymod(hlab, TWO_PI);
-            const float shifted = pymod(ga + half, TWO_PI);
-            int hc = (int)floorf(shifted / per);
-            hc = hc < 0 ? 0 : (hc > NB - 1 ? NB - 1 : hc);
-            const float hres = (shifted - ((float)hc * per + half)) / half;
-            {
-                float mx = o[3];
-                int am = 0;
-#pragma unroll
-                for (int j = 1; j < NB; ++j)
-                    if (o[3 + j] > mx) { mx = o[3 + j]; am = j; }
-                float se = 0.f, ej[NB];
-#pragma unroll
-                for (int j = 0; j < NB; ++j) { ej[j] = expf(o[3 + j] - mx); se += ej[j]; }
-                acc[3] += logf(se) + mx - o[3 + hc];
-#pragma unroll
-                for (int j = 0; j < NB; ++j) go[3 + j] += wB * (ej[j] / se - (j == hc ? 1.f : 0.f));
-                acc[9] += (am == hc) ? 1.f : 0.f;
-                const float e = o[3 + NB + hc] - hres;
-                const float ab = fabsf(e), q = fminf(ab, 1.f);
-                acc[4] += 0.5f * q * q + (ab - q);
-                go[3 + NB + hc] += wB * a.w_headreg * (e > 0.f ? q : (e < 0.f ? -q : 0.f));
-            }
-            {
-                const float *ss = &o[3 + 2 * NB];
-                float mx = ss[0];
-                int am = 0;
-#pragma unroll
-                for (int j = 1; j < NS; ++j)
-                    if (ss[j] > mx) { mx = ss[j]; am = j; }
-                float se = 0.f;
-#pragma unroll
-                for (int j = 0; j < NS; ++j) {
-                    const float ej = expf(ss[j] - mx);
-                    go[3 + 2 * NB + j] = ej;
-                    se += ej;
-                }
-                acc[5] += logf(se) + mx - ss[sc];
-#pragma unroll
-                for (int j = 0; j < NS; ++j) go[3 + 2 * NB + j] = wB * (go[3 + 2 * NB + j] / se - (j == sc ? 1.f : 0.f));
-                acc[10] += (am == sc) ? 1.f : 0.f;
-            }
-            const int so = 3 + 2 * NB + NS + sc * 3;
-            {
-                const float v0 = (sl0 - ex0) / ex0 - o[so], v1 = (sl1 - ex1) / ex1 - o[so + 1],
-                            v2 = (sl2 - ex2) / ex2 - o[so + 2];
-                const float n = sqrtf(v0 * v0 + v1 * v1 + v2 * v2);
-                const float q = fminf(n, 1.f);
-                acc[6] += 0.5f * q * q + (n - q);
-                if (n > 0.f) {
-                    const float k = -wB * a.w_sizereg * q / n;
-                    go[so] += k * v0; go[so + 1] += k * v1; go[so + 2] += k * v2;
-                }
-            }
-            {
-                float ang = (float)hc * per + o[3 + NB + hc] * half;
-                if (ang > PI) ang -= TWO_PI;
-                const float pl = o[so] * ex0 + ex0, pw = o[so + 1] * ex1 + ex1, ph = o[so + 2] * ex2 + ex2;
-                const float pcx = rx + o[0], pcy = ry + o[1], pcz = rz + o[2];
-                float px[8], py[8], pz[8], gx[8], gy[8], gz[8], fx[8], fy[8], fz[8];
-                const float c = cosf(ang), s = sinf(ang);
-                const float hf = hlab + PI;
-                corners8(pcx, pcy, pcz, c, s, pl, pw, ph, px, py, pz);
-                corners8(clx, cly, clz, cosf(hlab), sinf(hlab), sl0, sl1, sl2, gx, gy, gz);
-                corners8(clx, cly, clz, cosf(hf), sinf(hf), sl0, sl1, sl2, fx, fy, fz);
-                float d1 = 0.f, d2 = 0.f;
-#pragma unroll
-                for (int k = 0; k < 8; ++k) {
-                    d1 += sqrtf((px[k] - gx[k]) * (px[k] - gx[k]) + (py[k] - gy[k]) * (py[k] - gy[k]) +
-                                (pz[k] - gz[k]) * (pz[k] - gz[k]));
-                    d2 += sqrtf((px[k] - fx[k]) * (px[k] - fx[k]) + (py[k] - fy[k]) * (py[k] - fy[k]) +
-                                (pz[k] - fz[k]) * (pz[k] - fz[k]));
-                }
-                d1 *= 0.125f; d2 *= 0.125f;
-                const bool first = d1 <= d2;
-                const float cd = first ? d1 : d2;
-                const float q = fminf(cd, 1.f);
-                acc[7] += 0.5f * q * q + (cd - q);
-                const float wk = wB * a.w_corner * q * 0.125f;
-                float dcx = 0.f, dcy = 0.f, dcz = 0.f, dl = 0.f, dw = 0.f, dh = 0.f, dang = 0.f;
-#pragma unroll
-                for (int k = 0; k < 8; ++k) {
-                    const float tx = first ? gx[k] : fx[k], ty = first ? gy[k] : fy[k], tz = first ? gz[k] : fz[k];
-                    const float ex_ = px[k] - tx, ey_ = py[k] - ty, ez_ = pz[k] - tz;
-                    const float nn = sqrtf(ex_ * ex_ + ey_ * ey_ + ez_ * ez_);
-                    if (nn > 0.f) {
-                        const float kx = wk * ex_ / nn, ky = wk * ey_ / nn, kz = wk * ez_ / nn;
-                        const float sx = (k & 2) ? -0.5f : 0.5f, sy = (k & 4) ? -0.5f : 0.5f;
-                        const float sz = ((k & 3) == 1 || (k & 3) == 2) ? -0.5f : 0.5f;
-                        const float x = sx * pl, z = sz * pw;
-                        dcx += kx; dcy += ky; dcz += kz;
-                        dl += kx * c * sx - kz * s * sx;
-                        dw += kx * s * sz + kz * c * sz;
-                        dh += ky * sy;
-                        dang += kx * (-s * x + c * z) + kz * (-c * x - s * z);
-                    }
-                }
-                go[0] += dcx; go[1] += dcy; go[2] += dcz;
-                go[so] += dl * ex0; go[so + 1] += dw * ex1; go[so + 2] += dh * ex2;
-                go[3 + NB + hc] += dang * half;
-            }
-        }
-        if (a.ld) {
-        } else if (a.dreg) {
-#pragma unroll
-            for (int j = 0; j < NC; ++j) a.dreg[((int64_t)b * NC + j) * L2 + l] = go[j];
-        }
-    }
-    if (a.ld && a.dcls) {
-        __syncthreads();
-        for (int i = tid; i < nrow * q4; i += LT_THREADS) {
-            const int rr = i >> sh_q, c4 = i & (q4 - 1);
-            lt_v4f v;
-#pragma unroll
-            for (int j = 0; j < 4; ++j) v[j] = 4 * c4 + j < NC + 2 ? gG[rr * SW + 4 * c4 + j] : 0.f;
-            *(lt_v4f *)(a.dcls + (int64_t)(row0 + rr) * a.ld + 4 * c4) = v;
-        }
+        }
+    } else if (a.dreg && live) {
+#pragma unroll
+        for (int j = 0; j < NC; ++j) a.dreg[((int64_t)b * NC + j) * L2 + l] = gG[tid * SW + 2 + j];
     }
     float tot[11];
 #pragma unroll
     for (int i = 0; i < 11; ++i) tot[i] = acc[i];
     block_sums<LT_THREADS, 11>(tot, shN);
+    const LossWeights lw = {a.w_box, a.w_corner, a.w_headreg, a.w_sizereg};
+    if (a.scratch && a.defer) {
+        if (tid == 0) {
+#pragma unroll
+            for (int i = 1; i < 11; ++i) a.scratch[32 + 16 * blockIdx.x + i] = tot[i];
+            if (blockIdx.x == 0) {
+                a.scratch[1] = nfg; a.scratch[2] = nkeep;
+                ((int *)a.scratch)[3] = (int)gridDim.x; ((int *)a.scratch)[4] = TREF; ((int *)a.scratch)[5] = PAIR;
+            }
+        }
+        return;
+    }
     if (tid == 0) {
         int ticket;
         if (a.scratch) {
@@ -338,34 +383,16 @@
         last_s = (ticket == (int)gridDim.x - 1) ? 1 : 0;
     }
     __syncthreads();
-    if (last_s && a.scratch) {
+    if (!last_s) return;
+    if (a.scratch) {
         __threadfence();
-        float pt_[11];
-#pragma unroll
-        for (int i = 1; i < 11; ++i) pt_[i] = 0.f;
-        for (int g = tid; g < (int)gridDim.x; g += LT_THREADS)
-#pragma unroll
-            for (int i = 1; i < 11; ++i)
-                pt_[i] += __hip_atomic_load(&a.scratch[32 + 16 * g + i], __ATOMIC_RELAXED, __HIP_MEMORY_SCOPE_AGENT);
-#pragma unroll
-        for (int i = 1; i < 11; ++i) gG[tid * 11 + i] = pt_[i];
-    }
-    __syncthreads();
-    if (last_s && tid == 0) {
+        lt_combine(a.scratch, (int)gridDim.x, TREF, PAIR, nfg, nkeep, gG, a.out, a.total, lw, tid, LT_THREADS);
+        if (tid == 0) ((int *)a.scratch)[0] = 0;
+    } else if (tid == 0) {
         float t[11];
-        if (a.scratch) {
-#pragma unroll
-            for (int i = 1; i < 11; ++i) t[i] = 0.f;
-            const int nth = min((int)gridDim.x, LT_THREADS);
-            for (int g = 0; g < nth; ++g)
-#pragma unroll
-                for (int i = 1; i < 11; ++i) t[i] += gG[g * 11 + i];
-            ((int *)a.scratch)[0] = 0;
-        } else {
-            __threadfence();
-#pragma unroll
-            for (int i = 1; i < 11; ++i) t[i] = __hip_atomic_load(&a.out[i], __ATOMIC_RELAXED, __HIP_MEMORY_SCOPE_AGENT);
-        }
+        __threadfence();
+#pragma unroll
+        for (int i = 1; i < 11; ++i) t[i] = __hip_atomic_load(&a.out[i], __ATOMIC_RELAXED, __HIP_MEMORY_SCOPE_AGENT);
         const float cls = t[1] * inv_cls;
         const float center = t[2] * inv_fg, hcls = t[3] * inv_fg, hres = t[4] * inv_fg;
         const float scls = t[5] * inv_fg, sres = t[6] * inv_fg, corner = t[7] * inv_fg;
@@ -380,6 +407,10 @@
     }
 }
 
+#ifndef LT_NS3_THREADS
+#define LT_NS3_THREADS 64
+#endif
+
 static int launch_loss(const LossArgs &a, int ns, hipStream_t st)
 {
     if (!a.scratch) {
@@ -387,8 +418,10 @@
         if (e != hipSuccess) return (int)e;
     }
     const int R = a.B * a.L2;
-    if (ns == 3) hipLaunchKernelGGL((loss_tail_kernel<3, 128>), dim3((R + 127) / 128), dim3(128), 0, st, a);
-    else hipLaunchKernelGGL((loss_tail_kernel<10, 64>), dim3((R + 63) / 64), dim3(64), 0, st, a);
+    if (ns == 3)
+        hipLaunchKernelGGL((loss_tail_kernel<3, LT_NS3_THREADS, 128>), dim3((R + LT_NS3_THREADS - 1) / LT_NS3_THREADS),
+                           dim3(LT_NS3_THREADS), 0, st, a);
+    else hipLaunchKernelGGL((loss_tail_kernel<10, 64, 64>), dim3((R + 63) / 64), dim3(64), 0, st, a);
     FCN_CHECK_LAUNCH();
     return 0;
 }
@@ -411,7 +444,7 @@
     a.box_center = box3d_center; a.box_heading = box3d_heading; a.box_size = box3d_size; a.size_class = size_class;
     a.mean_size = mean_size; a.out = out16; a.dcls = dcls; a.dreg = dreg; a.B = B; a.L2 = L2;
     a.w_box = w_box; a.w_corner = w_corner; a.w_headreg = w_headreg; a.w_sizereg = w_sizereg; a.ld = 0;
-    a.scratch = nullptr; a.total = nullptr;
+    a.scratch = nullptr; a.total = nullptr; a.defer = 0;
     return launch_loss(a, num_size_cluster, (hipStream_t)stream);
 }
 
@@ -421,6 +454,12 @@
                                        int num_heading_bin, int num_size_cluster,
                                        float w_box, float w_corner, float w_headreg, float w_sizereg,
                                        float *out16, float *dlogits, float *scratch, float *total, void *stream);
+extern "C" int fcn_det_loss_tail_rows3(const float *logits, const int64_t *cls_label, const float *center_ref2,
+                                       const float *box3d_center, const float *box3d_heading, const float *box3d_size,
+                                       const int64_t *size_class, const float *mean_size, int B, int L2,
+                                       int num_heading_bin, int num_size_cluster,
+                                       float w_box, float w_corner, float w_headreg, float w_sizereg,
+                                       float *out16, float *dlogits, float *scratch, float *total, int defer, void *stream);
 
 extern "C" int fcn_det_loss_tail_rows(const float *logits, const int64_t *cls_label, const float *center_ref2,
                                       const float *box3d_center, const float *box3d_heading, const float *box3d_size,
@@ -446,9 +485,22 @@
                                        float w_box, float w_corner, float w_headreg, float w_sizereg,
                                        float *out16, float *dlogits, float *scratch, float *total, void *stream)
 {
+    return fcn_det_loss_tail_rows3(logits, cls_label, center_ref2, box3d_center, box3d_heading, box3d_size, size_class,
+                                   mean_size, B, L2, num_heading_bin, num_size_cluster, w_box, w_corner, w_headreg,
+                                   w_sizereg, out16, dlogits, scratch, total, 0, stream);
+}
+
+extern "C" int fcn_det_loss_tail_rows3(const float *logits, const int64_t *cls_label, const float *center_ref2,
+                                       const float *box3d_center, const float *box3d_heading, const float *box3d_size,
+                                       const int64_t *size_class, const float *mean_size, int B, int L2,
+                                       int num_heading_bin, int num_size_cluster,
+                                       float w_box, float w_corner, float w_headreg, float w_sizereg,
+                                       float *out16, float *dlogits, float *scratch, float *total, int defer, void *stream)
+{
     if (!logits || !cls_label || !center_ref2 || !box3d_center || !box3d_heading || !box3d_size || !size_class ||
-        !mean_size || !out16)
+        !mean_size || (!out16 && !defer))
         return FCN_E_BADARG;
+    if (defer && !scratch) return FCN_E_BADARG;
     if (num_heading_bin != LT_NB || (num_size_cluster != 3 && num_size_cluster != 10)) return FCN_E_LIMIT;
     if (B <= 0 || L2 <= 0) return FCN_E_BADARG;
     if (((uintptr_t)cls_label & 15) || ((uintptr_t)logits & 15) || ((uintptr_t)dlogits & 15)) return FCN_E_BADARG;
@@ -458,6 +510,6 @@
     a.mean_size = mean_size; a.out = out16; a.dcls = dlogits; a.dreg = nullptr; a.B = B; a.L2 = L2;
     a.w_box = w_box; a.w_corner = w_corner; a.w_headreg = w_headreg; a.w_sizereg = w_sizereg;
     a.ld = (2 + 3 + 2 * num_heading_bin + 4 * num_size_cluster <= 64) ? 64 : 128;
-    a.scratch = scratch; a.total = total;
+    a.scratch = scratch; a.total = total; a.defer = defer ? 1 : 0;
     return launch_loss(a, num_size_cluster, (hipStream_t)stream);
 }
diff --git a/frustum_convnet_amd/det_base.py b/frustum_convnet_amd/det_base.py
--- a/frustum_convnet_amd/det_base.py
+++ b/frustum_convnet_amd/det_base.py
@@ -649,19 +649,20 @@
                     size_probs.view(batch_size, -1, self.num_size_cluster))
 
         if fused_tail:
-            from .loss_fused import det_loss_tail, det_loss_tail_rows, loss_scratch
+            from .loss_fused import det_loss_tail, det_loss_tail_rows_deferred, loss_scratch
             Lw = cfg.LOSS
             wts = (Lw.BOX_LOSS_WEIGHT, Lw.CORNER_LOSS_WEIGHT, Lw.HEAD_REG_WEIGHT, Lw.SIZE_REG_WEIGHT)
             if logits64 is not None:
                 key = (batch_size, num_out, str(logits64.device))
                 if self._loss_scratch is None or self._loss_scratch[0] != key:
                     self._loss_scratch = (key, loss_scratch(batch_size, num_out, logits64.device))
-                ious = self._iou_metrics(logits64, batch_size, num_out, cls_label, refs[1], center_label, heading_label,
-                                         size_label, mean_size_array, self.num_bins, self.num_size_cluster, cfg.IOU_THRESH)
-                losses, (a_cls, a_head, a_size), nfg = det_loss_tail_rows(
+                losses, (a_cls, a_head, a_size), nfg, pending = det_loss_tail_rows_deferred(
                     logits64, batch_size, num_out, cls_label, refs[1], center_label, heading_label, size_label,
                     size_class_label, mean_size_array, self.num_bins, self.num_size_cluster, wts,
                     self._loss_scratch[1])
+                ious = self._iou_metrics(logits64, batch_size, num_out, cls_label, refs[1], center_label, heading_label,
+                                         size_label, mean_size_array, self.num_bins, self.num_size_cluster, cfg.IOU_THRESH,
+                                         finish=pending)
                 if not (self.defer_metrics_join and self._differentiates()):
                     self._iou_metrics.join()
                 iou2, iou3, iout = ious[0], ious[1], ious[2]
diff --git a/frustum_convnet_amd/loss_fused.py b/frustum_convnet_amd/loss_fused.py
--- a/frustum_convnet_amd/loss_fused.py
+++ b/frustum_convnet_amd/loss_fused.py
@@ -76,7 +76,7 @@
 class _LossTailRows(torch.autograd.Function):
 
     @staticmethod
-    def forward(ctx, logits, cls_label, ref2, center, heading, size, size_class, mean_size, B, L2, nb, ns, w, scratch):
+    def forward(ctx, logits, cls_label, ref2, center, heading, size, size_class, mean_size, B, L2, nb, ns, w, scratch, defer=False):
         L = _native.lib()
         _check_labels(cls_label, size_class, ns)
         lg = logits.detach().contiguous()
@@ -88,12 +88,12 @@
                 heading.contiguous().float(), size.contiguous().float(), size_class.contiguous(),
                 mean_size.contiguous().float()]
         with torch.cuda.device(lg.device):
-            rc = L.fcn_det_loss_tail_rows2(lg.data_ptr(), *[t.data_ptr() for t in args], int(B), int(L2), int(nb),
+            rc = L.fcn_det_loss_tail_rows3(lg.data_ptr(), *[t.data_ptr() for t in args], int(B), int(L2), int(nb),
                                            int(ns), float(w[0]), float(w[1]), float(w[2]), float(w[3]),
                                            out.data_ptr(), None if dlog is None else dlog.data_ptr(),
                                            None if scratch is None else scratch.data_ptr(), total.data_ptr(),
-                                           _native.current_stream(lg.device))
-        _native.check(rc, "fcn_det_loss_tail_rows2")
+                                           1 if defer else 0, _native.current_stream(lg.device))
+        _native.check(rc, "fcn_det_loss_tail_rows3")
         ctx.need = need
         if need:
             ctx.save_for_backward(dlog)
@@ -104,9 +104,9 @@
     @staticmethod
     def backward(ctx, gtotal, _grest):
         if not ctx.need or gtotal is None:
-            return (None,) * 14
+            return (None,) * 15
         (dlog,) = ctx.saved_tensors
-        return (dlog if _is_unit(gtotal) else dlog * gtotal,) + (None,) * 13
+        return (dlog if _is_unit(gtotal) else dlog * gtotal,) + (None,) * 14
 
 
 def loss_scratch(B, L2, device):
@@ -124,6 +124,16 @@
     return losses, (rest[8], rest[9], rest[10]), rest[11]
 
 
+def det_loss_tail_rows_deferred(logits, B, L2, cls_label, center_ref2, box3d_center, box3d_heading, box3d_size, size_class,
+                                mean_size, num_bins, num_sizes, weights, scratch):
+    total, rest = _LossTailRows.apply(logits, cls_label, center_ref2, box3d_center, box3d_heading, box3d_size,
+                                      size_class, mean_size, B, L2, num_bins, num_sizes, weights, scratch, True)
+    losses = {"total_loss": total}
+    for i, k in enumerate(LOSS_NAMES[1:], start=1):
+        losses[k] = rest[i]
+    return losses, (rest[8], rest[9], rest[10]), rest[11], (scratch, rest, total, tuple(float(x) for x in weights))
+
+
 class IouMetrics:
 
     def __init__(self):
@@ -131,7 +141,7 @@
         self._join = None
 
     def __call__(self, logits, B, L2, cls_label, center_ref2, box3d_center, box3d_heading, box3d_size, mean_size, num_bins,
-                 num_sizes, iou_thresh):
+                 num_sizes, iou_thresh, finish=None):
         dev = logits.device
         key = str(dev)
         if key not in self.per_dev:
@@ -151,12 +161,17 @@
         side.wait_event(ev_in)
         with torch.cuda.stream(side):
             with torch.cuda.device(dev):
-                rc = _native.lib().fcn_det_iou_metrics(lg.data_ptr(), int(lg.shape[1]), *[t.data_ptr() for t in args], int(B),
-                                                       int(L2), int(num_bins), int(num_sizes), float(iou_thresh),
-                                                       scratch.data_ptr(), out.data_ptr(), _native.current_stream(dev))
-            _native.check(rc, "fcn_det_iou_metrics")
+                if finish is None:
+                    fin, held = [None, None, None, 0.0, 0.0, 0.0, 0.0], []
+                else:
+                    ls, lo, lt, lw = finish
+                    fin, held = [ls.data_ptr(), lo.data_ptr(), lt.data_ptr()] + list(lw), [ls, lo.detach(), lt.detach()]
+                rc = _native.lib().fcn_det_iou_metrics2(lg.data_ptr(), int(lg.shape[1]), *[t.data_ptr() for t in args], int(B),
+                                                        int(L2), int(num_bins), int(num_sizes), float(iou_thresh),
+                                                        scratch.data_ptr(), out.data_ptr(), *fin, _native.current_stream(dev))
+            _native.check(rc, "fcn_det_iou_metrics2")
             ev_out.record(side)
-        for t in [lg, out] + args:
+        for t in [lg, out] + args + held:
             t.record_stream(side)
         self._join = (cur, ev_out)
         return out
diff --git a/include/fcn_hip.h b/include/fcn_hip.h
--- a/include/fcn_hip.h
+++ b/include/fcn_hip.h
@@ -195,12 +195,23 @@
                             int num_heading_bin, int num_size_cluster,
                             float w_box, float w_corner, float w_headreg, float w_sizereg,
                             float *out16, float *dlogits, float *scratch, float *total, void *stream);
+int fcn_det_loss_tail_rows3(const float *logits, const int64_t *cls_label, const float *center_ref2,
+                            const float *box3d_center, const float *box3d_heading, const float *box3d_size,
+                            const int64_t *size_class, const float *mean_size, int B, int L2,
+                            int num_heading_bin, int num_size_cluster,
+                            float w_box, float w_corner, float w_headreg, float w_sizereg,
+                            float *out16, float *dlogits, float *scratch, float *total, int defer, void *stream);
 
 int fcn_box3d_iou_pair_f32(const float *corners1, const float *corners2, int n, float *out2, void *stream);
 int fcn_det_iou_metrics(const float *logits, int ld, const int64_t *cls_label, const float *center_ref2,
                         const float *box3d_center, const float *box3d_heading, const float *box3d_size,
                         const float *mean_size, int B, int L2, int num_heading_bin, int num_size_cluster,
                         float iou_thresh, float *scratch8, float *out4, void *stream);
+int fcn_det_iou_metrics2(const float *logits, int ld, const int64_t *cls_label, const float *center_ref2,
+                         const float *box3d_center, const float *box3d_heading, const float *box3d_size,
+                         const float *mean_size, int B, int L2, int num_heading_bin, int num_size_cluster,
+                         float iou_thresh, float *scratch8, float *out4, const float *loss_scratch, float *loss_out16,
+                         float *loss_total, float w_box, float w_corner, float w_headreg, float w_sizereg, void *stream);
 int fcn_decode_detections(const float *logits, int ld, const float *center_ref2, const float *mean_size,
                           const float *rot_angle, const float *ref_center, const float *rgb_prob, int B, int L2,
                           int num_heading_bin, int num_size_cluster, int method, float *dets, int32_t *valid,
```

New measurement: 29800 frustums/s (median of 6 runs). Within noise of the previous version (+0.4%).
